# JGI-Bioinformatics/Kmernator

Hardware: AMD Instinct MI355X
Metric: total k-mers/sec at k=31, 150 bp reads (spectrum build, inputs resident in HBM) (higher is better)
Workload: dtype u64

## Files before the change

### kmernator_amd/csrc/kmr_api.hip

```cpp
#include <hip/hip_runtime.h>
#include <dlfcn.h>
#include <unistd.h>
#include <rccl/rccl.h>

#include <algorithm>
#include <atomic>
#include <cmath>
#include <cstdio>
#include <cstdlib>
#include <cstring>
#include <cctype>
#include <memory>
#include <mutex>
#include <string>
#include <type_traits>
#include <vector>

#include "kmr_host.hpp"
#include "kmr_kernels.hpp"
#include "kmr_partition.hpp"
#include "kmr_superkmer.hpp"
#include "kmr_buckets.hpp"
#include "kmr_synth.hpp"
#define KMR_INSTANCES_EXTERN
// ... 84 lines not shown
	HIPCHK(h, hipGetLastError());
	return 0;
}
int clear_table_any(kmr_handle *h, void *slots, ExtSlot *ext, uint32_t log2cap) { return with_w(h, [&](auto W) { return clear_table<W()>(h, slots, ext, log2cap); }); }

int alloc_table(kmr_handle *h, uint32_t log2cap, DevBuf &slots, DevBuf &ext) {
	DevBuf s, x;
	HIPCHK(h, s.alloc(slot_bytes(h) << log2cap));
	if (h->ext) HIPCHK(h, x.alloc(sizeof(ExtSlot) << log2cap));
	const int rc = clear_table_any(h, s.get(), x.get<ExtSlot>(), log2cap);
	if (rc) return rc;
	slots = std::move(s); ext = std::move(x);
	return 0;
}

int sync_state(kmr_handle *h) {
	HIPCHK(h, hipStreamSynchronize(h->stream));
	for (int which = 0; which < KMR_TIME_GROUPS; which++) {
		for (auto &pr : h->pending_events[which]) {
			float ms = 0; hipEventElapsedTime(&ms, pr.first, pr.second);
			h->ms[which] += ms; h->launches[which]++;
			hipEventDestroy(pr.first); hipEventDestroy(pr.second);
		}
		h->pending_events[which].clear();
	}
	uint32_t e = 0; DevStats s;
	HIPCHK(h, hipMemcpy(&e, h->derr.get<uint32_t>(), sizeof(e), hipMemcpyDeviceToHost));
	HIPCHK(h, hipMemcpy(&s, h->dstats.get<DevStats>(), sizeof(s), hipMemcpyDeviceToHost));
#ifdef KMR_DEBUG_HOOKS
	if (h->superkmer_mode) { if (dbg()) fprintf(stderr, "sk_extract windows: %llu general, %llu fast\n", s.claimed, s.inserted); s.claimed = 0; s.inserted = 0; }
#endif
	h->stats.raw_kmers = s.raw + s.inserted + s.sender_bad; h->stats.raw_good_kmers = s.good + s.inserted; h->stats.discarded = s.raw - s.good + s.sender_bad;
	h->occupied = s.claimed; h->pending_kmers = 0; h->subtracted = s.subtracted;
	if (e & ERR_READ_TOO_LONG) return fail(h, KMR_ERR_UNSUPPORTED, "a read is longer than the per-wavefront LDS tile (" + std::to_string(TILE_SPAN) + " bases)");
	if (e & ERR_TABLE_FULL) return fail(h, KMR_ERR_CAPACITY, "device k-mer table is full; raise kmr_config.max_table_entries / estimated_raw_kmers");
	if (e & ERR_SEGMENT_OVERFLOW) return fail(h, KMR_ERR_CAPACITY, "an owner segment overflowed seg_capacity");
	if (e & ERR_POOL_FULL) return fail(h, KMR_ERR_CAPACITY, "record pool overflow (internal sizing error)");
	if (e & ERR_ENTRIES_FULL) return fail(h, KMR_ERR_CAPACITY, "entry buffer overflow (internal sizing error)");
	return 0;
}

template <int W, bool EXT> int grow_table_t(kmr_handle *h, uint32_t newlog) {
	DevBuf ns, ne;
	int rc = alloc_table(h, newlog, ns, ne);
	if (rc) return rc;
	Table<W> src = table_of<W>(h), dst; dst.slots = ns.get<Slot<W>>(); dst.ext = ne.get<ExtSlot>(); dst.log2cap = newlog;
	hipLaunchKernelGGL((rehash_kernel<W, EXT>), dim3(grid_for(1ull << h->log2cap)), dim3(256), 0, h->stream, src, dst, h->hkb, h->derr.get<uint32_t>());
	HIPCHK(h, hipGetLastError());
	HIPCHK(h, hipStreamSynchronize(h->stream));
	h->slots = std::move(ns); h->extslots = std::move(ne); h->log2cap = newlog;
	return 0;
}
int grow_table(kmr_handle *h, uint32_t newlog) { return with_w_ext(h, [&](auto W, auto EXT) { return grow_table_t<W(), EXT()>(h, newlog); }); }

int ensure_capacity(kmr_handle *h, uint64_t incoming) {
	const uint64_t cap = 1ull << h->log2cap;
	if ((double)(h->occupied + h->pending_kmers + incoming) <= 0.85 * (double)cap) { h->pending_kmers += incoming; return 0; }
	int rc = sync_state(h);
	if (rc) return rc;
	if ((double)(h->occupied + incoming) > 0.85 * (double)cap) {
		uint32_t nl = h->log2cap;
		while ((double)(h->occupied + incoming) > 0.6 * (double)(1ull << nl)) nl++;
		rc = grow_table(h, nl);
		if (rc) return rc;
	}
	h->pending_kmers = incoming;
	return 0;
}

void time_begin(kmr_handle *h, int which, hipEvent_t *a, hipEvent_t *b) {
	hipEventCreate(a); hipEventCreate(b);
	hipEventRecord(*a, h->stream);
	(void)which;
}
void time_end(kmr_handle *h, int which, hipEvent_t a, hipEvent_t b) {
	hipEventRecord(b, h->stream);
	h->pending_events[which].push_back(std::make_pair(a, b));
}

const size_t EXTRACT_SMEM = (size_t)WAVES_PER_BLOCK * 2 * TILE_BUF;

int prepare_units(kmr_handle *h, ReadsView &rv, uint32_t span = (uint32_t)TILE_SPAN) {
	rv.u_start = rv.u_end = rv.u_read = nullptr; rv.n_units = 0;
	const uint64_t n = rv.n_reads;
	if (n == 0) return 0;
	int rc = h->umax.reserve(h, "umax", 4); if (rc) return rc;
	HIPCHK(h, hipMemsetAsync(h->umax.get<unsigned int>(), 0, 4, h->stream));
	rc = h->ucnt.reserve(h, "ucnt", 4 * (n + 1)); if (rc) return rc;
	hipLaunchKernelGGL(unit_count_kernel, dim3(grid_for(n)), dim3(256), 0, h->stream, rv.offsets, n, h->k, span, h->ucnt.get<uint32_t>(), h->umax.get<unsigned int>());
	HIPCHK(h, hipGetLastError());
	unsigned int mx = 0;
	HIPCHK(h, hipMemcpyAsync(&mx, h->umax.get<unsigned int>(), 4, hipMemcpyDeviceToHost, h->stream));
	HIPCHK(h, hipStreamSynchronize(h->stream));
	if (mx <= span) return 0;
	rc = h->ufirst.reserve(h, "ufirst", 8 * (n + 1)); if (rc) return rc;
	rc = exclusive_scan(h, h->ucnt.get<uint32_t>(), n, h->ufirst.get<uint64_t>()); if (rc) return rc;
	uint64_t U = 0;
	HIPCHK(h, hipMemcpy(&U, h->ufirst.get<uint64_t>() + n, 8, hipMemcpyDeviceToHost));
	if (h->u_read.cap() < 8 * U) {
		h->u_start.reset(); h->u_end.reset(); h->u_read.reset();
		HIPCHK(h, h->u_start.alloc(8 * U)); HIPCHK(h, h->u_end.alloc(8 * U)); HIPCHK(h, h->u_read.alloc(8 * U));
	}
	hipLaunchKernelGGL(unit_fill_kernel, dim3(grid_for(n)), dim3(256), 0, h->stream, rv.offsets, n, h->k, span, h->ufirst.get<uint64_t>(), h->u_start.get<uint64_t>(), h->u_end.get<uint64_t>(), h->u_read.get<uint64_t>());
	HIPCHK(h, hipGetLastError());
	rv.u_start = h->u_start.get<uint64_t>(); rv.u_end = h->u_end.get<uint64_t>(); rv.u_read = h->u_read.get<uint64_t>(); rv.n_units = U;
	return 0;
}

template <int W, bool EXT, class Op> int launch_extract(kmr_handle *h, const ReadsView &rv, const Op &op, uint64_t max_blocks = 0) {
	const DevParams dp = dev_params(h);
	const bool sub = Op::NEEDS_WEIGHT && (dp.sub_wnb | dp.sub_snb) != 0;
	auto kern = sub ? extract_kernel<W, EXT, Op, true> : extract_kernel<W, EXT, Op, false>;
	HIPCHK(h, hipFuncSetAttribute((const void *)kern, hipFuncAttributeMaxDynamicSharedMemorySize, (int)EXTRACT_SMEM));
	if (dbg()) { int nb = 0; hipOccupancyMaxActiveBlocksPerMultiprocessor(&nb, (const void *)kern, WAVES_PER_BLOCK * 64, EXTRACT_SMEM); fprintf(stderr, "extract: %d blocks of %d waves per CU (dynamic LDS %zu)\n", nb, WAVES_PER_BLOCK, EXTRACT_SMEM);
		for (size_t tr : {(size_t)79872, (size_t)65536, (size_t)52000, (size_t)38000}) { hipOccupancyMaxActiveBlocksPerMultiprocessor(&nb, (const void *)kern, WAVES_PER_BLOCK * 64, tr); fprintf(stderr, "   with %zu bytes: %d blocks\n", tr, nb); } }
	const uint64_t tiles = ((rv.u_start ? rv.n_units : rv.n_reads) + 63) / 64;
	uint64_t blocks = (tiles + WAVES_PER_BLOCK - 1) / WAVES_PER_BLOCK;
	if (blocks == 0) return 0;
	if (max_blocks && blocks > max_blocks) blocks = max_blocks;
	if (blocks > 0x7fffffffull) return fail(h, KMR_ERR_INVALID_ARG, "too many reads in one batch");
	hipLaunchKernelGGL(kern, dim3((unsigned)blocks), dim3(WAVES_PER_BLOCK * 64), EXTRACT_SMEM, h->stream, rv, dp, op);
	HIPCHK(h, hipGetLastError());
	return 0;
}

template <int W, bool EXT> int add_reads_dev_t(kmr_handle *h, const ReadsView &rvAll, uint64_t total_bases) {
	const uint64_t n = rvAll.n_reads;
	const uint64_t avg = n ? std::max<uint64_t>(1, total_bases / n) : 1;
	uint64_t chunk = std::max<uint64_t>(64, ((1ull << 27) / avg) & ~63ull);
	std::vector<uint64_t> off2(2);
	for (uint64_t r = 0; r < n; r += chunk) {
		const uint64_t m = std::min(chunk, n - r);
		HIPCHK(h, hipMemcpyAsync(&off2[0], rvAll.offsets + r, 8, hipMemcpyDeviceToHost, h->stream));
		HIPCHK(h, hipMemcpyAsync(&off2[1], rvAll.offsets + r + m, 8, hipMemcpyDeviceToHost, h->stream));
		HIPCHK(h, hipStreamSynchronize(h->stream));
		const uint64_t bases = off2[1] - off2[0];
		int rc = ensure_capacity(h, bases);
		if (rc) return rc;
		ReadsView rv = reads_slice(rvAll, r, m);
		rc = prepare_units(h, rv); if (rc) return rc;
		InsertOp<W, EXT> op; op.table = table_of<W>(h);
		hipEvent_t a, b; time_begin(h, 0, &a, &b);
		rc = launch_extract<W, EXT>(h, rv, op);
		time_end(h, 0, a, b);
		if (rc) return rc;
	}
	return 0;
}

int add_reads_dev_any(kmr_handle *h, const ReadsView &rv, uint64_t total_bases) { return with_w_ext(h, [&](auto W, auto EXT) { return add_reads_dev_t<W(), EXT()>(h, rv, total_bases); }); }

}
namespace kmr_host {
int exclusive_scan(kmr_handle *h, const uint32_t *in, uint64_t n, uint64_t *out ) {
	const uint64_t nblocks = (n + SCAN_ITEMS - 1) / SCAN_ITEMS;
	const size_t eb = sizeof(unsigned long long);
	int rc = h->scan_sums.reserve(h, "scan_sums", eb * (nblocks + 1), eb * std::max<uint64_t>(nblocks + 1, 4096)); if (rc) return rc;
	unsigned long long *sums = h->scan_sums.get<unsigned long long>(), *total = sums + nblocks;
	hipLaunchKernelGGL(scan_block_sums_kernel, dim3((unsigned)nblocks), dim3(256), 0, h->stream, in, n, sums);
	hipLaunchKernelGGL(scan_sums_kernel, dim3(1), dim3(256), 0, h->stream, sums, nblocks, total);
	hipLaunchKernelGGL(scan_apply_kernel, dim3((unsigned)nblocks), dim3(256), 0, h->stream, in, n, sums, out);
	HIPCHK(h, hipGetLastError());
	HIPCHK(h, hipStreamSynchronize(h->stream));
	return 0;
}
}
namespace {

int arena_alloc(kmr_handle *h, void **out, size_t bytes) {
	const size_t need = (bytes + 255) & ~(size_t)255;
	if (h->arena && h->arena_used + need <= h->arena.cap()) { *out = h->arena.get<uint8_t>() + h->arena_used; h->arena_used += need; h->arena_want += need; return 0; }
	h->arena_want += need;
	DevBuf b;
	HIPCHK(h, b.alloc(std::max<size_t>(need, 256)));
	*out = b.get();
	h->arena_overflow.push_back(std::move(b));
	return 0;
}
int arena_reset(kmr_handle *h) {
	HIPCHK(h, hipStreamSynchronize(h->stream));
	h->arena_overflow.clear();
	if (h->arena_want > h->arena.cap()) {
		if (h->arena.alloc(h->arena_want + h->arena_want / 8 + (1 << 20)) != hipSuccess) (void)hipGetLastError();
	}
	h->arena_used = 0; h->arena_want = 0;
	return 0;
}
template <class T> int arena_get(kmr_handle *h, T **out, size_t count) { return arena_alloc(h, (void **)out, count * sizeof(T)); }

void clear_map(DevMap &m) { m.image.reset(); m.n = 0; m.present = false; }


template <int W> MapView<W> view_of(const DevMap &m, uint32_t vw) {
	MapView<W> v; v.start = m.start.get<uint64_t>(); v.keys = m.keys.get<uint64_t>(); v.vals = m.vals.get<uint32_t>(); v.sweight = m.sweight.get<uint8_t>(); v.nb = m.present ? m.nb : 0; v.vw = vw;
	return v;
}

template <int W, bool EXT> int finalize_t(kmr_handle *h, uint32_t min_depth) {
	int rc = sync_state(h);
	if (rc) return rc;
	hipEvent_t ea, eb; time_begin(h, 1, &ea, &eb);
	const FinalizeParams f = finalize_params(h, min_depth);
	const bool keepSing = f.has_singletons && min_depth <= 1;
	DevBuf wcb, scb, fcb;
	HIPCHK(h, wcb.alloc(4 * h->nb_weak)); HIPCHK(h, scb.alloc(4 * h->nb_sing)); HIPCHK(h, fcb.alloc(sizeof(FinalizeCounters)));
	uint32_t *wc = wcb.get<uint32_t>(), *sc = scb.get<uint32_t>(); FinalizeCounters *fc = fcb.get<FinalizeCounters>();
	HIPCHK(h, hipMemsetAsync(wc, 0, 4 * h->nb_weak, h->stream)); HIPCHK(h, hipMemsetAsync(sc, 0, 4 * h->nb_sing, h->stream)); HIPCHK(h, hipMemsetAsync(fc, 0, sizeof(FinalizeCounters), h->stream));
	Table<W> t = table_of<W>(h);
	const int g = grid_for(1ull << h->log2cap);
	hipLaunchKernelGGL(classify_kernel<W>, dim3(g), dim3(256), 0, h->stream, t, f, wc, sc, fc);
	HIPCHK(h, hipGetLastError());
	FinalizeCounters c;
	HIPCHK(h, hipMemcpyAsync(&c, fc, sizeof(c), hipMemcpyDeviceToHost, h->stream));
	HIPCHK(h, hipStreamSynchronize(h->stream));
	h->stats.unique_kmers = c.unique;
	h->stats.singleton_kmers = f.has_singletons ? c.singletons : 0;
	DevMap &wm = h->weak, &sm = h->sing;
	wm = DevMap(); sm = DevMap();
	wm.nb = h->nb_weak; wm.n = c.weak_kept; wm.present = true;
	sm.nb = h->nb_sing; sm.n = c.sing_kept; sm.present = keepSing;
	const uint32_t vw = EXT ? 15 : 3;
	HIPCHK(h, wm.start.alloc(8 * (wm.nb + 1))); HIPCHK(h, sm.start.alloc(8 * (sm.nb + 1)));
	rc = exclusive_scan(h, wc, wm.nb, wm.start.get<uint64_t>()); if (rc) return rc;
	rc = exclusive_scan(h, sc, sm.nb, sm.start.get<uint64_t>()); if (rc) return rc;
	HIPCHK(h, wm.keys.alloc(std::max<uint64_t>(8, 8ull * W * wm.n))); HIPCHK(h, wm.vals.alloc(std::max<uint64_t>(8, 4ull * vw * wm.n)));
	HIPCHK(h, sm.keys.alloc(std::max<uint64_t>(8, 8ull * W * sm.n))); HIPCHK(h, sm.sweight.alloc(std::max<uint64_t>(8, sm.n)));
	if (EXT) HIPCHK(h, sm.spkt.alloc(std::max<uint64_t>(8, 4ull * sm.n)));
	HIPCHK(h, hipMemsetAsync(wc, 0, 4 * h->nb_weak, h->stream)); HIPCHK(h, hipMemsetAsync(sc, 0, 4 * h->nb_sing, h->stream));
	hipLaunchKernelGGL((scatter_kernel<W, EXT>), dim3(g), dim3(256), 0, h->stream, t, f, wm.start.get<uint64_t>(), wc, wm.keys.get<uint64_t>(), wm.vals.get<uint32_t>(), sm.start.get<uint64_t>(), sc, sm.keys.get<uint64_t>(), sm.sweight.get<uint8_t>(), sm.spkt.get<uint32_t>());
	HIPCHK(h, hipGetLastError());
	SortView<W> sv; sv.keys = wm.keys.get<uint64_t>(); sv.vals = wm.vals.get<uint32_t>(); sv.b8 = nullptr; sv.pkt = nullptr; sv.vw = vw;
	hipLaunchKernelGGL((sort_buckets_kernel<W, EXT ? 15 : 3>), dim3(grid_for(wm.nb, 4, 1 << 20)), dim3(256), 0, h->stream, sv, wm.start.get<uint64_t>(), wm.nb);
	if (sm.n) {
		SortView<W> ss; ss.keys = sm.keys.get<uint64_t>(); ss.vals = nullptr; ss.b8 = sm.sweight.get<uint8_t>(); ss.pkt = sm.spkt.get<uint32_t>(); ss.vw = 0;
		hipLaunchKernelGGL((sort_buckets_kernel<W, 0>), dim3(grid_for(sm.nb, 4, 1 << 20)), dim3(256), 0, h->stream, ss, sm.start.get<uint64_t>(), sm.nb);
	}
	HIPCHK(h, hipGetLastError());
	time_end(h, 1, ea, eb);
	HIPCHK(h, hipStreamSynchronize(h->stream));
	h->has_singletons = keepSing;
	if (!keepSing) { sm.n = 0; }
	h->stats.weak_entries = wm.n; h->stats.singleton_entries = keepSing ? sm.n : 0;
	h->finalized = true; h->map_gen++;
	return sync_state(h);
}

template <int W> int build_image_t(kmr_handle *h, DevMap &m, bool weakMap) {
	if (m.image) return 0;
	const uint32_t vw = h->ext ? 15 : 3;
	const uint32_t vbytes = weakMap ? (h->ext ? 60 : 12) : (h->ext ? 5 : 1);
	HIPCHK(h, m.image.alloc(8 * (2 + m.nb) + 4 * m.nb + m.n * (h->kb + vbytes)));
	hipLaunchKernelGGL(image_header_kernel, dim3(grid_for(m.nb)), dim3(256), 0, h->stream, m.image.get<uint8_t>(), m.start.get<uint64_t>(), m.nb, h->kb, vbytes);
	if (m.n) hipLaunchKernelGGL(image_entries_kernel<W>, dim3(grid_for(m.n)), dim3(256), 0, h->stream, m.image.get<uint8_t>(), m.start.get<uint64_t>(), m.nb, h->kb, vbytes,
	                           m.keys.get<uint64_t>(), weakMap ? m.vals.get<uint32_t>() : nullptr, vw, m.sweight.get<uint8_t>(), m.spkt.get<uint32_t>(), m.n);
	HIPCHK(h, hipGetLastError());
	HIPCHK(h, hipStreamSynchronize(h->stream));
	return 0;
}
int build_image(kmr_handle *h, DevMap &m, bool weakMap) { return with_w(h, [&](auto W) { return build_image_t<W()>(h, m, weakMap); }); }

template <int W> int load_image_t(kmr_handle *h, DevMap &m, bool weakMap, const uint8_t *src, uint64_t len) {
	if (len < 16) return fail(h, KMR_ERR_INVALID_ARG, "image too short");
	uint64_t nb, mask; memcpy(&nb, src, 8); memcpy(&mask, src + 8, 8);
	if (nb == 0 || (nb & (nb - 1)) || mask != nb - 1 || len < 8 * (2 + nb) + 4 * nb) return fail(h, KMR_ERR_INVALID_ARG, "bad image header");
	const uint32_t vw = h->ext ? 15 : 3;
	const uint32_t vbytes = weakMap ? (h->ext ? 60 : 12) : (h->ext ? 5 : 1);
	if ((len - 8 * (2 + nb) - 4 * nb) % (h->kb + vbytes) != 0) return fail(h, KMR_ERR_INVALID_ARG, "image size does not match k / value type");
	m = DevMap();
	m.nb = nb; m.n = (len - 8 * (2 + nb) - 4 * nb) / (h->kb + vbytes); m.present = true;
	const uint64_t *offs = (const uint64_t *)(src + 16);
	uint64_t expect = 8 * (2 + nb);
	for (uint64_t b = 0; b < nb; b++) {
		if (offs[b] != expect || expect + 4 > len) return fail(h, KMR_ERR_INVALID_ARG, "image offsets are not the packed store() layout");
		uint32_t cnt; memcpy(&cnt, src + expect, 4);
		expect += 4 + (uint64_t)cnt * (h->kb + vbytes);
		if (expect > len) return fail(h, KMR_ERR_INVALID_ARG, "image bucket runs past the end");
	}
	if (expect != len) return fail(h, KMR_ERR_INVALID_ARG, "image length mismatch");
	HIPCHK(h, m.image.alloc(len));
	HIPCHK(h, hipMemcpy(m.image.get<uint8_t>(), src, len, hipMemcpyHostToDevice));
	{
		DevBuf counts; HIPCHK(h, counts.alloc(4 * nb));
		hipLaunchKernelGGL(image_counts_kernel, dim3(grid_for(nb)), dim3(256), 0, h->stream, m.image.get<uint8_t>(), nb, counts.get<uint32_t>());
		HIPCHK(h, m.start.alloc(8 * (nb + 1)));
		int rc = exclusive_scan(h, counts.get<uint32_t>(), nb, m.start.get<uint64_t>()); if (rc) return rc;
	}
	HIPCHK(h, m.keys.alloc(std::max<uint64_t>(8, 8ull * W * m.n)));
	if (weakMap) HIPCHK(h, m.vals.alloc(std::max<uint64_t>(8, 4ull * vw * m.n)));
	else { HIPCHK(h, m.sweight.alloc(std::max<uint64_t>(8, m.n))); if (h->ext) HIPCHK(h, m.spkt.alloc(std::max<uint64_t>(8, 4 * m.n))); }
	if (m.n) hipLaunchKernelGGL(image_unpack_kernel<W>, dim3(grid_for(m.n)), dim3(256), 0, h->stream, m.image.get<uint8_t>(), m.start.get<uint64_t>(), nb, h->kb, vbytes, m.keys.get<uint64_t>(), m.vals.get<uint32_t>(), vw, m.sweight.get<uint8_t>(), m.spkt.get<uint32_t>(), m.n);
	SortView<W> sv; sv.keys = m.keys.get<uint64_t>(); sv.vals = m.vals.get<uint32_t>(); sv.b8 = m.sweight.get<uint8_t>(); sv.pkt = m.spkt.get<uint32_t>(); sv.vw = weakMap ? vw : 0;
	if (!weakMap) hipLaunchKernelGGL((sort_buckets_kernel<W, 0>), dim3(grid_for(nb, 4, 1 << 20)), dim3(256), 0, h->stream, sv, m.start.get<uint64_t>(), nb);
	else if (h->ext) hipLaunchKernelGGL((sort_buckets_kernel<W, 15>), dim3(grid_for(nb, 4, 1 << 20)), dim3(256), 0, h->stream, sv, m.start.get<uint64_t>(), nb);
	else hipLaunchKernelGGL((sort_buckets_kernel<W, 3>), dim3(grid_for(nb, 4, 1 << 20)), dim3(256), 0, h->stream, sv, m.start.get<uint64_t>(), nb);
	HIPCHK(h, hipGetLastError());
	HIPCHK(h, hipStreamSynchronize(h->stream));
	m.image.reset();

	return 0;
}

template <int W, int VW> void launch_sort(kmr_handle *h, DevMap &m, bool weakMap) {
	SortView<W> sv; sv.keys = m.keys.get<uint64_t>(); sv.vals = weakMap ? m.vals.get<uint32_t>() : nullptr; sv.b8 = m.sweight.get<uint8_t>(); sv.pkt = m.spkt.get<uint32_t>(); sv.vw = weakMap ? VW : 0;
	hipLaunchKernelGGL((sort_buckets_kernel<W, VW>), dim3(grid_for(m.nb, 4, 1 << 20)), dim3(256), 0, h->stream, sv, m.start.get<uint64_t>(), m.nb);
}
template <int W> int merge_image_t(kmr_handle *h, DevMap &m, bool weakMap, const uint8_t *src, uint64_t len) {
	DevMap t;
	int rc = load_image_t<W>(h, t, weakMap, src, len);
	if (rc) return rc;
	if (t.nb != m.nb) return fail(h, KMR_ERR_INVALID_ARG, "Can not merge two maps of differing sizes (src/Kmer.h:3210)");
	const uint32_t vw = h->ext ? 15 : 3;
	DevMap d; d.nb = m.nb; d.n = m.n + t.n; d.present = true;
	DevBuf countsb, dupb;
	HIPCHK(h, countsb.alloc(4 * m.nb)); HIPCHK(h, dupb.alloc(4));
	uint32_t *counts = countsb.get<uint32_t>(), *dup = dupb.get<uint32_t>();
// ... 198 lines not shown
				HIPCHK(h, hipStreamSynchronize(h->stream));
				h->uw_keys.reset(); h->uw_vals.reset(); h->us_keys.reset(); h->us_b8.reset(); h->us_pkt.reset(); h->ue.reset(); h->ue2.reset();
			}
		}
		uint64_t want = est / CH + launches * (uint64_t)grid * ((1ull << h->bits1) + 512) + 64 + l2_allowance;
		{
			size_t mfree = 0, mtotal = 0;
			const double twice = (double)(want + est / CH) * CH * rec_bytes(h) * 1.02;
			if (hipMemGetInfo(&mfree, &mtotal) == hipSuccess && twice + (double)(8ull << 30) < (double)mfree * 0.5) want += est / CH;
		}
		int rc0 = pool_reserve(h, h->l1, want, true);
		if (rc0) return rc0;
	}
	int rc = pool_reserve(h, h->l1, max_records / CH + (uint64_t)grid * ((1ull << h->bits1) + 512) + 64, true);
	if (rc) return rc;
	rc = zero_work_counter(h); if (rc) return rc;
	PartSource<W> S; memset(&S, 0, sizeof(S));
	S.linear = linear; S.ext_start = ext_start; S.ext_count = ext_count; S.n_ext = n_ext; S.ext_stride = ext_stride; S.ext_len = ext_len; S.total = total;
	S.valid_counter = valid_counter; S.kb = h->hkb; S.rot = part_rot(h); S.packed_words = packed_words; S.ordinal_base = ordinal_base;
	if (!h->tune.no_l1_state) {
		rc = ensure_l1_state<W, EXT>(h); if (rc) return rc;
		S.state = h->l1_state.get<uint8_t>(); S.state_final = 0; h->l1_state_dirty = true;
	}
	hipEvent_t ta, tb; time_begin(h, KMR_TIME_PARTITION1, &ta, &tb);
	rc = launch_partition<W, EXT, 1>(h, S, h->l1, grid, h->bits1, 0);
	time_end(h, KMR_TIME_PARTITION1, ta, tb);
	return rc;
}

void choose_bits1(kmr_handle *h, uint64_t records_hint) {
	uint64_t est = std::max<uint64_t>(records_hint, h->cfg.estimated_raw_kmers / std::max<uint32_t>(1, h->cfg.world_size));
	const int mb = max_part_bits(h);
	int T = 0; while (T < 2 * mb && (est >> T) > TARGET_LIST_RECORDS) T++;
	h->bits1 = std::max(0, std::min(mb, T + 2 - mb));
}

template <int W, bool EXT> int extract_by_owner_t(kmr_handle *h, const ReadsView &rvAll, uint64_t total_bases, void *dev_records, uint64_t seg_capacity, void *dev_seg_counts, uint32_t *dev_pos = nullptr) {
	const uint64_t n = rvAll.n_reads;
	const uint64_t avg = n ? std::max<uint64_t>(1, total_bases / n) : 1;
	const uint64_t chunk = std::max<uint64_t>(64, (SUB_BATCH_BASES / avg) & ~63ull);
	for (uint64_t r = 0; r < n; r += chunk) {
		const uint64_t m = std::min(chunk, n - r);
		ReadsView rv = reads_slice(rvAll, r, m);
		int rc = prepare_units(h, rv); if (rc) return rc;
		const uint64_t nu = rv.u_start ? rv.n_units : m;
		rc = h->kcap.reserve(h, "kcap", 4 * std::max<uint64_t>(nu + 1, 16)); if (rc) return rc;
		rc = h->koff.reserve(h, "koff", 8 * std::max<uint64_t>(nu + 1, 16)); if (rc) return rc;
		hipLaunchKernelGGL(kmer_capacity_kernel, dim3(grid_for(nu)), dim3(256), 0, h->stream, rv, h->k, h->kcap.get<uint32_t>());
		HIPCHK(h, hipGetLastError());
		rc = exclusive_scan(h, h->kcap.get<uint32_t>(), nu, h->koff.get<uint64_t>()); if (rc) return rc;
		uint64_t total_cap = 0;
		HIPCHK(h, hipMemcpy(&total_cap, h->koff.get<uint64_t>() + nu, 8, hipMemcpyDeviceToHost));
		const uint64_t tiles = (nu + 63) / 64;
		rc = h->linear.reserve(h, "linear", sizeof(typename PoolRec<W, EXT>::type) * std::max<uint64_t>(total_cap, 16)); if (rc) return rc;
		rc = h->tile_count.reserve(h, "tile_count", 4 * std::max<uint64_t>(tiles, 16)); if (rc) return rc;
		LinearOp<W, EXT, false> op; op.records = (typename PoolRec<W, EXT>::type *)h->linear.get(); op.koff = h->koff.get<uint64_t>(); op.tile_count = h->tile_count.get<uint32_t>(); op.first_read_idx = rv.first_read_idx;
		h->sender_launch = dev_pos == nullptr;
		rc = launch_extract<W, EXT>(h, rv, op);
		h->sender_launch = false;
		if (rc) return rc;
		rc = zero_work_counter(h); if (rc) return rc;
		const int grid = (int)std::min<uint64_t>((uint64_t)num_cus(h) * 8, tiles);
		OwnerFn of; of.m = 0; of.off = of.win = of.list_bits = 0;
		if (h->superkmer_mode && h->sk_exchange) { of.m = h->sk_m; of.off = h->sk_off; of.win = h->sk_win; of.list_bits = h->sk_bits; }
		if (dev_pos)
			hipLaunchKernelGGL((owner_scatter_kernel<W, EXT, true>), dim3(grid), dim3(OWNER_THREADS), 0, h->stream, (const typename PoolRec<W, EXT>::type *)h->linear.get(), h->koff.get<uint64_t>(), h->tile_count.get<uint32_t>(), tiles, h->hkb,
			                   h->cfg.world_size, (uint32_t *)dev_records, seg_capacity, (unsigned long long *)dev_seg_counts, h->work_counter.get<unsigned int>(), h->derr.get<uint32_t>(), dev_pos, of);
		else
			hipLaunchKernelGGL((owner_scatter_kernel<W, EXT>), dim3(grid), dim3(OWNER_THREADS), 0, h->stream, (const typename PoolRec<W, EXT>::type *)h->linear.get(), h->koff.get<uint64_t>(), h->tile_count.get<uint32_t>(), tiles, h->hkb,
			                   h->cfg.world_size, (uint32_t *)dev_records, seg_capacity, (unsigned long long *)dev_seg_counts, h->work_counter.get<unsigned int>(), h->derr.get<uint32_t>(), (uint32_t *)nullptr, of);
		HIPCHK(h, hipGetLastError());
	}
	return 0;
}

template <int W, bool EXT> int add_reads_partition_t(kmr_handle *h, const ReadsView &rvAll, uint64_t total_bases) {
	const uint64_t n = rvAll.n_reads;
	if (!h->l1.head) choose_bits1(h, total_bases);
	const uint64_t avg = n ? std::max<uint64_t>(1, total_bases / n) : 1;
	const uint64_t sub_bases = h->tune.sub_batch_bases ? h->tune.sub_batch_bases : SUB_BATCH_BASES;
	const uint64_t chunk = std::max<uint64_t>(64, (sub_bases / avg) & ~63ull);
	for (uint64_t r = 0; r < n; r += chunk) {
		const uint64_t m = std::min(chunk, n - r);
		ReadsView rv = reads_slice(rvAll, r, m);
		int rc = prepare_units(h, rv); if (rc) return rc;
		const uint64_t nu = rv.u_start ? rv.n_units : m;
		rc = h->kcap.reserve(h, "kcap", 4 * std::max<uint64_t>(nu + 1, 16)); if (rc) return rc;
		rc = h->koff.reserve(h, "koff", 8 * std::max<uint64_t>(nu + 1, 16)); if (rc) return rc;
		hipLaunchKernelGGL(kmer_capacity_kernel, dim3(grid_for(nu)), dim3(256), 0, h->stream, rv, h->k, h->kcap.get<uint32_t>());
		HIPCHK(h, hipGetLastError());
		rc = exclusive_scan(h, h->kcap.get<uint32_t>(), nu, h->koff.get<uint64_t>()); if (rc) return rc;
		uint64_t total_cap = 0;
		HIPCHK(h, hipMemcpy(&total_cap, h->koff.get<uint64_t>() + nu, 8, hipMemcpyDeviceToHost));
		const uint64_t tiles = (nu + 63) / 64;
		rc = h->linear.reserve(h, "linear", rec_bytes(h) * std::max<uint64_t>(total_cap, 16)); if (rc) return rc;
		rc = h->tile_count.reserve(h, "tile_count", 4 * std::max<uint64_t>(tiles, 16)); if (rc) return rc;
		LinearOp<W, EXT> op; op.records = (typename PoolRec<W, EXT>::type *)h->linear.get(); op.koff = h->koff.get<uint64_t>(); op.tile_count = h->tile_count.get<uint32_t>(); op.first_read_idx = rv.first_read_idx;
		hipEvent_t a, b, a2, b2; time_begin(h, KMR_TIME_BUILD, &a, &b);
		time_begin(h, KMR_TIME_EXTRACT, &a2, &b2);
		rc = launch_extract<W, EXT>(h, rv, op);
		time_end(h, KMR_TIME_EXTRACT, a2, b2);
#ifdef KMR_DEBUG_HOOKS
		if (!rc && getenv("KMR_DEBUG_SAME_TILE")) {
			const uint64_t distinct = std::max<uint64_t>(1, strtoull(getenv("KMR_DEBUG_SAME_TILE"), nullptr, 10));
			hipLaunchKernelGGL(same_tile_kernel, dim3(grid_for(tiles)), dim3(256), 0, h->stream, h->koff.get<uint64_t>(), tiles, distinct, total_cap / std::max<uint64_t>(tiles, 1));
		}
#endif
		if (!rc) rc = partition_level1<W, EXT>(h, h->linear.get(), h->koff.get<uint64_t>(), h->tile_count.get<uint32_t>(), tiles, 64, 0, 0, total_cap);
		time_end(h, KMR_TIME_BUILD, a, b);
		if (rc) return rc;
	}
	return 0;
}
int add_reads_partition(kmr_handle *h, const ReadsView &rv, uint64_t total_bases) { return with_w_ext(h, [&](auto W, auto EXT) { return add_reads_partition_t<W(), EXT()>(h, rv, total_bases); }); }

int build_csr(kmr_handle *h, HostPool &p, uint64_t nl, uint32_t first, uint64_t **list_start, uint64_t **list_chunks, uint32_t *n_chunks_out) {
	unsigned int used = 0;
	HIPCHK(h, hipStreamSynchronize(h->stream));
	HIPCHK(h, hipMemcpy(&used, p.head.get<unsigned int>(), 4, hipMemcpyDeviceToHost));
	if (used > p.cap) used = p.cap;
	used = used > first ? used - first : 0;
	uint32_t *cnt;
	{ int arc = arena_get(h, &cnt, nl); if (arc) return arc; arc = arena_get(h, list_start, nl + 1); if (arc) return arc;
	  arc = arena_get(h, list_chunks, std::max<unsigned>(used, 1)); if (arc) return arc; }
	HIPCHK(h, hipMemsetAsync(cnt, 0, 4 * nl, h->stream));
	const unsigned csr_grid = (unsigned)(((uint64_t)used + CSR_THREADS * CSR_ITEMS - 1) / (CSR_THREADS * CSR_ITEMS));
	if (used) hipLaunchKernelGGL(chunk_hist_kernel, dim3(csr_grid), dim3(CSR_THREADS), 0, h->stream, p.chunk_list.get<uint32_t>() + first, used, cnt, (uint32_t)nl);
	int rc = exclusive_scan(h, cnt, nl, *list_start); if (rc) return rc;
	HIPCHK(h, hipMemsetAsync(cnt, 0, 4 * nl, h->stream));
	if (used) hipLaunchKernelGGL(chunk_scatter_kernel, dim3(csr_grid), dim3(CSR_THREADS), 0, h->stream, p.chunk_list.get<uint32_t>() + first, p.chunk_count.get<uint32_t>() + first, used, first, *list_start, cnt, *list_chunks, (uint32_t)nl);
	HIPCHK(h, hipGetLastError());
	*n_chunks_out = used;
	if (dbg()) {
		unsigned long long hv[2] = {0, 0};
		DevBuf db; HIPCHK(h, db.alloc(16)); HIPCHK(h, hipMemset(db.get(), 0, 16));
		unsigned long long *d = db.get<unsigned long long>();
		if (used) hipLaunchKernelGGL(pool_records_kernel, dim3(grid_for(used)), dim3(256), 0, h->stream, p.chunk_list.get<uint32_t>(), p.chunk_count.get<uint32_t>(), used, d, d + 1);
		HIPCHK(h, hipStreamSynchronize(h->stream));
		HIPCHK(h, hipMemcpy(hv, d, 16, hipMemcpyDeviceToHost));
		fprintf(stderr, "build_csr: lists %llu chunks %u valid %llu records %llu (expected %llu)\n", (unsigned long long)nl, used, hv[1], hv[0], (unsigned long long)h->stats.raw_good_kmers);
		unsigned long long vv[3] = {0, 0, 0};
		int bits = 0; while ((1ull << bits) < nl) bits++;
		DevBuf vb; HIPCHK(h, vb.alloc(24)); HIPCHK(h, hipMemset(vb.get(), 0, 24));
		unsigned long long *v = vb.get<unsigned long long>();
		PoolView pvw = pool_view(h, p);
		with_w_ext(h, [&](auto W, auto EXT) { hipLaunchKernelGGL((verify_lists_kernel<W(), EXT()>), dim3(4096), dim3(256), 0, h->stream, pvw, *list_start, *list_chunks, nl, bits, h->hkb, part_rot(h), v, v + 1, v + 2); });
		HIPCHK(h, hipStreamSynchronize(h->stream));
		HIPCHK(h, hipMemcpy(vv, v, 24, hipMemcpyDeviceToHost));
		fprintf(stderr, "verify_lists: records via CSR %llu misfiled %llu zero-weight %llu\n", vv[0], vv[1], vv[2]);
	}
	return 0;
}

int finish_maps_from_entries(kmr_handle *h, uint32_t *wc, uint32_t *sc, uint64_t wslots, uint64_t sslots, uint64_t wn, uint64_t sn, bool keepSing, bool weak_uncounted = false);
CountOut count_out(kmr_handle *h, bool packed, unsigned long long *cursors, uint32_t *wc, uint32_t *sc, FinalizeCounters *fc);

template <int W, bool EXT, int LOG2S, bool NARROW = false> int launch_count(kmr_handle *h, int grid, const uint64_t *ls, const uint64_t *lc, uint64_t nl, const CountOut &out, const FinalizeParams &f, int list_filter) {
	auto kern = count_kernel<W, EXT, LOG2S, NARROW>;
	const size_t smem = count_smem_bytes<W, EXT, LOG2S, NARROW>();
	HIPCHK(h, hipFuncSetAttribute((const void *)kern, hipFuncAttributeMaxDynamicSharedMemorySize, (int)smem));
	hipLaunchKernelGGL(kern, dim3(grid), dim3(COUNT_THREADS), smem, h->stream, pool_view(h, h->l1), ls, lc, nl, out, f, h->work_counter.get<unsigned int>(), list_filter);
	return 0;
}

template <int W, bool EXT> int finalize_partition_t(kmr_handle *h, uint32_t min_depth) {
	int rc = sync_state(h);
	if (rc) return rc;
	hipEvent_t ea, eb; time_begin(h, 1, &ea, &eb);
	const uint64_t G = h->stats.raw_good_kmers;
	const FinalizeParams f = finalize_params(h, min_depth);
	const bool keepSing = f.has_singletons && min_depth <= 1;
	if (!h->l1.head) { rc = pool_reserve(h, h->l1, 0, false); if (rc) return rc; }
	rc = arena_reset(h); if (rc) return rc;
	rc = flush_l1_state<W, EXT>(h); if (rc) return rc;
	const uint64_t nl1 = 1ull << h->bits1;
	uint64_t *ls1 = nullptr; uint64_t *lc1 = nullptr; uint32_t nch1 = 0;
	rc = build_csr(h, h->l1, nl1, 0, &ls1, &lc1, &nch1); if (rc) return rc;
	double distinct_share = 1.0, repeated_share = 0.5;
	if (G) {
		unsigned long long *dpr, hpr[4] = {0, 0, 0, 0};
		const uint32_t n_probes = (uint32_t)std::min<uint64_t>(PROBE_LISTS, nl1);
		const size_t tbytes = 8 * ((size_t)n_probes * PROBE_SLOTS + 4);
		rc = arena_alloc(h, (void **)&dpr, tbytes); if (rc) return rc;
		HIPCHK(h, hipMemsetAsync(dpr, 0, tbytes, h->stream));
		hipLaunchKernelGGL((distinct_probe_kernel<W, EXT>), dim3(n_probes * PROBE_SPLIT), dim3(256), 0, h->stream, pool_view(h, h->l1), ls1, lc1, nl1, h->hkb, part_rot(h),
		                   (int)h->bits1, n_probes, dpr + 4, dpr);
		HIPCHK(h, hipGetLastError());
		HIPCHK(h, hipMemcpyAsync(hpr, dpr, 32, hipMemcpyDeviceToHost, h->stream)); HIPCHK(h, hipStreamSynchronize(h->stream));
		if (hpr[0] >= 256) { distinct_share = std::min(1.0, std::max(0.01, (double)hpr[1] / (double)hpr[0])); repeated_share = std::min(0.5, (double)hpr[2] / (double)hpr[0]); }
		if (dbg()) fprintf(stderr, "distinct probe: %llu records, %llu distinct (%llu repeated) -> shares %.3f %.3f\n", hpr[0], hpr[1], hpr[2], distinct_share, repeated_share);
	}
	const int mb = max_part_bits(h);
	int T = 0; while (T < 40 && ((G >> T) > TARGET_LIST_RECORDS || (double)(G >> T) * distinct_share > MAX_LIST_DISTINCT)) T++;
	T = std::min(T, 28);
	int cur_bits = h->bits1;
	uint64_t *ls2 = ls1, *lc2 = lc1;
	uint32_t valid_from = 0;
	for (int level = 2; cur_bits < T; level++) {
		const int nbits = std::min(mb, T - cur_bits);
		const uint64_t nl_prev = 1ull << cur_bits;
		std::vector<uint64_t> hs(nl_prev + 1);
		HIPCHK(h, hipMemcpy(hs.data(), ls2, 8 * (nl_prev + 1), hipMemcpyDeviceToHost));
		std::vector<uint64_t> ib, ie; std::vector<uint32_t> il;
		for (uint64_t l = 0; l < nl_prev; l++) {
			const uint64_t nch = hs[l + 1] - hs[l];
			if (!nch) continue;
			const uint64_t nit = (nch + L2_ITEM_CHUNKS - 1) / L2_ITEM_CHUNKS, per = (nch + nit - 1) / nit;
			for (uint64_t c = hs[l]; c < hs[l + 1]; c += per) { ib.push_back(c); ie.push_back(std::min(hs[l + 1], c + per)); il.push_back((uint32_t)l); }
		}
		if (ib.empty()) { cur_bits += nbits; rc = build_csr(h, h->l1, 1ull << cur_bits, valid_from, &ls2, &lc2, &nch1); if (rc) return rc; continue; }
		const uint64_t partials = ib.size() * (1ull << nbits) + (uint64_t)part_grid(h) * 512 + 64;
		unsigned int head_before = 0;
		HIPCHK(h, hipMemcpy(&head_before, h->l1.head.get<unsigned int>(), 4, hipMemcpyDeviceToHost));
		const bool recycle = h->tune.recycle >= 0 ? h->tune.recycle != 0 : (uint64_t)head_before + G / CH + partials + 64 > h->l1.cap;
		h->l1.used_ub = head_before;
		rc = pool_reserve(h, h->l1, (recycle ? 0 : G / CH) + partials, true); if (rc) return rc;
		uint64_t *dib, *die; uint32_t *dil;
		rc = arena_get(h, &dib, ib.size()); if (rc) return rc; rc = arena_get(h, &die, ie.size()); if (rc) return rc; rc = arena_get(h, &dil, il.size()); if (rc) return rc;
		HIPCHK(h, hipMemcpyAsync(dib, ib.data(), 8 * ib.size(), hipMemcpyHostToDevice, h->stream)); HIPCHK(h, hipMemcpyAsync(die, ie.data(), 8 * ie.size(), hipMemcpyHostToDevice, h->stream));
		HIPCHK(h, hipMemcpyAsync(dil, il.data(), 4 * il.size(), hipMemcpyHostToDevice, h->stream));
		rc = zero_work_counter(h); if (rc) return rc;
		PartSource<W> S; memset(&S, 0, sizeof(S));
		S.src = pool_view(h, h->l1); S.list_chunks = lc2; S.item_begin = dib; S.item_end = die; S.item_list = dil; S.n_items = ib.size(); S.kb = h->hkb; S.rot = part_rot(h);
		S.recycle = recycle ? 1 : 0;
		const int grid = (int)std::min<uint64_t>(partition_blocks(h), ib.size());
		if (dbg()) fprintf(stderr, "level %d: %d bits after %d, %zu items, %s\n", level, nbits, cur_bits, ib.size(), recycle ? "recycling chunks" : "fresh chunks");
		hipEvent_t ta, tb; time_begin(h, KMR_TIME_PARTITION2, &ta, &tb);
		rc = launch_partition<W, EXT, 2>(h, S, h->l1, grid, nbits, cur_bits);
		time_end(h, KMR_TIME_PARTITION2, ta, tb);
		if (rc) return rc;
		HIPCHK(h, hipStreamSynchronize(h->stream));
		cur_bits += nbits;
		if (!recycle) valid_from = head_before;
		rc = build_csr(h, h->l1, 1ull << cur_bits, valid_from, &ls2, &lc2, &nch1); if (rc) return rc;
	}
	const uint64_t nl2 = 1ull << cur_bits;
	const int count_log2s = (!EXT && (double)(G >> cur_bits) * distinct_share > MAX_LIST_DISTINCT) ? 11 : COUNT_LOG2S;
	if (dbg()) fprintf(stderr, "count pass: %llu lists of ~%llu records, table 2^%d\n", (unsigned long long)nl2, (unsigned long long)(G >> cur_bits), count_log2s);
	const uint32_t vw = EXT ? 15 : 3;
	const uint64_t slack = (uint64_t)part_grid(h) * 8 * 8192 + 16;
	const uint64_t wbound = f.has_singletons ? G / 2 : G, sbound = keepSing ? G : 0;
	const uint64_t wmax = wbound + wbound / 8 + slack, smax = keepSing ? sbound + sbound / 8 + slack : 16;
	uint64_t wcap = std::min<uint64_t>(wmax, (uint64_t)((double)G * (f.has_singletons ? repeated_share : distinct_share) * 1.5) + G / 64 + slack);
	uint64_t scap = keepSing ? std::min<uint64_t>(smax, (uint64_t)((double)G * std::max(0.0, distinct_share - repeated_share) * 1.5) + G / 64 + slack) : 16;
	if (h->tune.entry_share >= 0) {
		const double sh = h->tune.entry_share;
		wcap = std::min<uint64_t>(wmax, (uint64_t)((double)G * sh) + 16384); if (keepSing) scap = std::min<uint64_t>(smax, (uint64_t)((double)G * sh) + 16384);
		h->uw_keys.reset(); h->uw_vals.reset(); h->us_keys.reset(); h->us_b8.reset(); h->us_pkt.reset();
	}
	wcap = std::max(wcap, key_entries(h, h->uw_keys)); scap = std::max(scap, key_entries(h, h->us_keys));
	uint32_t *wc = nullptr, *sc = nullptr; FinalizeCounters *fc = nullptr; unsigned long long *cursors = nullptr;
	rc = arena_get(h, &wc, h->nb_weak); if (rc) return rc; rc = arena_get(h, &sc, h->nb_sing); if (rc) return rc;
	rc = arena_get(h, &fc, 1); if (rc) return rc; rc = arena_get(h, &cursors, 2); if (rc) return rc;
	FinalizeCounters c; unsigned long long cur[2];
	hipEvent_t tca, tcb; time_begin(h, KMR_TIME_COUNT, &tca, &tcb);
	for (int attempt = 0; ; attempt++) {
	{
		const double need = (key_entries(h, h->uw_keys) < wcap ? (8.0 * W + 4.0 * vw) * (double)wcap : 0.0) + (key_entries(h, h->us_keys) < scap ? (8.0 * W + 1.0) * (double)scap : 0.0);
		size_t mfree = 0, mtotal = 0;
		if (need > 0 && h->linear && hipMemGetInfo(&mfree, &mtotal) == hipSuccess && (double)mfree < need + (double)G * 0.3 * (8.0 * W + 12.0) + (double)(2ull << 30)) {
			HIPCHK(h, hipStreamSynchronize(h->stream));
			h->linear.reset();
		}
	}
	if (key_entries(h, h->uw_keys) < wcap || !h->uw_vals) {
		h->uw_keys.reset(); h->uw_vals.reset();
		HIPCHK(h, h->uw_keys.alloc(8ull * W * wcap)); HIPCHK(h, h->uw_vals.alloc(4ull * vw * wcap));
	}
	if (key_entries(h, h->us_keys) < scap || !h->us_b8 || (EXT && !h->us_pkt)) {
		h->us_keys.reset(); h->us_b8.reset(); h->us_pkt.reset();
		HIPCHK(h, h->us_keys.alloc(8ull * W * scap)); HIPCHK(h, h->us_b8.alloc(scap)); if (EXT) HIPCHK(h, h->us_pkt.alloc(4 * scap));
	}
	HIPCHK(h, hipMemsetAsync(wc, 0, 4 * h->nb_weak, h->stream)); HIPCHK(h, hipMemsetAsync(sc, 0, 4 * h->nb_sing, h->stream));
	HIPCHK(h, hipMemsetAsync(fc, 0, sizeof(FinalizeCounters), h->stream)); HIPCHK(h, hipMemsetAsync(cursors, 0, 16, h->stream));
	const CountOut out = count_out(h, false, cursors, wc, sc, fc);
	rc = zero_work_counter(h); if (rc) return rc;
	#ifdef KMR_DEBUG_HOOKS
	const int count_reps = getenv("KMR_COUNT_CHECK") ? atoi(getenv("KMR_COUNT_CHECK")) : 0;
#else
	const int count_reps = 0;
#endif
	for (int cr = 0; cr <= count_reps; cr++) {
		if (cr) {
			FinalizeCounters c0; unsigned long long cur0[2];
			HIPCHK(h, hipStreamSynchronize(h->stream));
			HIPCHK(h, hipMemcpy(&c0, fc, sizeof(c0), hipMemcpyDeviceToHost)); HIPCHK(h, hipMemcpy(cur0, cursors, 16, hipMemcpyDeviceToHost));
			fprintf(stderr, "count pass %d: unique %llu singletons %llu weak_kept %llu sing_kept %llu slots %llu/%llu\n", cr - 1, (unsigned long long)c0.unique,
			        (unsigned long long)c0.singletons, (unsigned long long)c0.weak_kept, (unsigned long long)c0.sing_kept, cur0[0], cur0[1]);
			HIPCHK(h, hipMemsetAsync(wc, 0, 4 * h->nb_weak, h->stream)); HIPCHK(h, hipMemsetAsync(sc, 0, 4 * h->nb_sing, h->stream));
			HIPCHK(h, hipMemsetAsync(fc, 0, sizeof(FinalizeCounters), h->stream)); HIPCHK(h, hipMemsetAsync(cursors, 0, 16, h->stream));
			rc = zero_work_counter(h); if (rc) return rc;
		}
		const int grid = (int)std::min<uint64_t>((uint64_t)part_grid(h) * 2, nl2);
		if (count_log2s == 11) {
			rc = launch_count<W, EXT, 11>(h, grid, ls2, lc2, nl2, out, f, 0); if (rc) return rc;
		} else if (EXT && W == 1 && !h->tune.no_narrow) {
			rc = launch_count<W, EXT, COUNT_LOG2S, true>(h, grid, ls2, lc2, nl2, out, f, 1); if (rc) return rc;
			HIPCHK(h, hipGetLastError());
			rc = zero_work_counter(h); if (rc) return rc;
			hipLaunchKernelGGL(max_list_chunks_kernel, dim3(grid_for(nl2)), dim3(256), 0, h->stream, ls2, nl2, h->work_counter.get<unsigned int>());
			unsigned int longest = 0;
			HIPCHK(h, hipMemcpyAsync(&longest, h->work_counter.get<unsigned int>(), 4, hipMemcpyDeviceToHost, h->stream));
			HIPCHK(h, hipStreamSynchronize(h->stream));
			rc = zero_work_counter(h); if (rc) return rc;
			if (longest > COUNT_NARROW_CHUNKS) { rc = launch_count<W, EXT, COUNT_LOG2S>(h, std::min(grid, part_grid(h)), ls2, lc2, nl2, out, f, 2); if (rc) return rc; }
		} else {
			rc = launch_count<W, EXT, COUNT_LOG2S>(h, grid, ls2, lc2, nl2, out, f, 0); if (rc) return rc;
		}
		HIPCHK(h, hipGetLastError());
	}
	uint32_t cerr = 0;
	HIPCHK(h, hipMemcpyAsync(&c, fc, sizeof(c), hipMemcpyDeviceToHost, h->stream)); HIPCHK(h, hipMemcpyAsync(cur, cursors, 16, hipMemcpyDeviceToHost, h->stream));
	HIPCHK(h, hipMemcpyAsync(&cerr, h->derr.get<uint32_t>(), 4, hipMemcpyDeviceToHost, h->stream));
	HIPCHK(h, hipStreamSynchronize(h->stream));
	if (!(cerr & ERR_ENTRIES_FULL) || (wcap >= wmax && scap >= smax) || attempt >= 8) break;
	cerr &= ~(uint32_t)ERR_ENTRIES_FULL;
	HIPCHK(h, hipMemcpy(h->derr.get<uint32_t>(), &cerr, 4, hipMemcpyHostToDevice));
	wcap = std::min<uint64_t>(wmax, wcap * 2); if (keepSing) scap = std::min<uint64_t>(smax, scap * 2);
	if (dbg()) fprintf(stderr, "count pass: entry buffers too small, retrying with %llu / %llu\n", (unsigned long long)wcap, (unsigned long long)scap);
	}
	time_end(h, KMR_TIME_COUNT, tca, tcb);
	{
		uint32_t cerr2 = 0;
		HIPCHK(h, hipMemcpy(&cerr2, h->derr.get<uint32_t>(), 4, hipMemcpyDeviceToHost));
		if (cerr2 & ERR_ENTRIES_FULL) { time_end(h, 1, ea, eb); return fail(h, KMR_ERR_CAPACITY, "entry buffers of the count pass overflowed at their upper bound (internal sizing error)"); }
	}

	h->stats.unique_kmers = c.unique;
	h->stats.singleton_kmers = f.has_singletons ? c.singletons : 0;
	hipEvent_t tma, tmb; time_begin(h, KMR_TIME_BUCKETS, &tma, &tmb);
	rc = finish_maps_from_entries(h, wc, sc, cur[0], cur[1], c.weak_kept, c.sing_kept, keepSing);
	time_end(h, KMR_TIME_BUCKETS, tma, tmb);
	if (rc) return rc;
	time_end(h, 1, ea, eb);
	h->has_singletons = keepSing;
	h->stats.weak_entries = h->weak.n; h->stats.singleton_entries = keepSing ? h->sing.n : 0;
	h->finalized = true; h->map_gen++;
	rc = sync_state(h);
	if (!rc && !h->arena_overflow.empty()) rc = arena_reset(h);
	return rc;
}

template <int W> int binned_buckets_t(kmr_handle *h, uint64_t wslots, uint64_t wn, bool &done) {
	done = false;
	DevMap &wm = h->weak;
	const uint64_t nb = wm.nb;
	uint32_t B = 0; while ((1ull << (B + 1)) <= nb) B++;
	if (h->ext || wn < h->tune.binned_min || wn == 0 || (1ull << B) != nb || wslots >= (1ull << 40)) return 0;
	uint32_t g = 0; while (g < std::min<uint32_t>(B, BB_MAX_GROUP_BITS) && (wn >> (B - g)) < 512) g++;
	const uint32_t R = B - g;
	if (R < 1 || R > 2 * BB_MAX_BITS || (wn >> R) > 1024) return 0;
	const uint32_t bits1 = R <= (uint32_t)BB_MAX_BITS ? R : (R + 1) / 2, bits2 = R - bits1;
	const uint64_t bins1 = 1ull << bits1, groups = 1ull << R;
	uint32_t *hist1 = nullptr, *hist2 = nullptr, *pad1 = nullptr; uint64_t *start1 = nullptr, *gstart = nullptr; unsigned long long *cursor = nullptr; unsigned int *dmax = nullptr;
	int rc = arena_get(h, &hist1, bins1); if (rc) return rc;
	rc = arena_get(h, &start1, bins1 + 1); if (rc) return rc;
	rc = arena_get(h, &cursor, groups); if (rc) return rc;
	rc = arena_get(h, &dmax, 1); if (rc) return rc;
	if (bits2) { rc = arena_get(h, &hist2, groups); if (rc) return rc; rc = arena_get(h, &pad1, bins1); if (rc) return rc; rc = arena_get(h, &gstart, groups + 1); if (rc) return rc; }
	HIPCHK(h, hipMemsetAsync(hist1, 0, 4 * bins1, h->stream)); HIPCHK(h, hipMemsetAsync(dmax, 0, 4, h->stream));
	BbInput in1; in1.entries = h->ue.get<uint64_t>(); in1.seg_start = nullptr; in1.seg_count = nullptr; in1.n_seg = 1; in1.n_slots = wslots; in1.holes = 1;
	auto hist_grid = [&](uint64_t n_slots, uint32_t &tpb) { const uint64_t tiles = (n_slots + BB_TILE - 1) / BB_TILE; tpb = (uint32_t)std::max<uint64_t>(1, (tiles + 2047) / 2048); return (unsigned)((tiles + tpb - 1) / tpb); };
	auto scatter_grid = [&](uint64_t n_slots) { const uint64_t tiles = (n_slots + BB_TILE - 1) / BB_TILE; return (unsigned)std::min<uint64_t>(tiles, (uint64_t)num_cus(h) * 8); };
	auto scratch = [&](uint64_t entries) { return h->ue2.reserve(h, "ue2", 8ull * (W + 1) * entries); };
	auto group_launch = [&](const uint64_t *entries, const uint64_t *gs, const uint32_t *gc) -> int {
		int rc2 = wm.keys.reserve(h, "weak map keys", std::max<uint64_t>(8ull * W * wn, 8)); if (rc2) return rc2;
		rc2 = wm.vals.reserve(h, "weak map vals", std::max<uint64_t>(12ull * wn, 8)); if (rc2) return rc2;
		auto gk = bb_group_kernel<W>;
		HIPCHK(h, hipFuncSetAttribute((const void *)gk, hipFuncAttributeMaxDynamicSharedMemorySize, (int)bb_group_smem_bytes<W>()));
		int per_cu = 0;
		if (hipOccupancyMaxActiveBlocksPerMultiprocessor(&per_cu, (const void *)gk, BB_GROUP_THREADS, bb_group_smem_bytes<W>()) != hipSuccess || per_cu < 1) per_cu = 4;
		if (dbg()) fprintf(stderr, "bb_group<W=%d>: %d blocks per CU, %llu groups\n", W, per_cu, (unsigned long long)groups);
		hipLaunchKernelGGL(gk, dim3((unsigned)std::min<uint64_t>(groups, (uint64_t)num_cus(h) * per_cu)), dim3(BB_GROUP_THREADS), bb_group_smem_bytes<W>(), h->stream, entries, wm.keys.get<uint64_t>(), wm.vals.get<uint32_t>(), gs, gc, groups, g, h->hkb, nb, wm.start.get<uint64_t>(), wn, h->derr.get<uint32_t>());
		HIPCHK(h, hipGetLastError());
		return 0;
	};
	const uint32_t shift1 = B - bits1;
	uint32_t tpb = 1; unsigned grid = hist_grid(wslots, tpb);
	hipLaunchKernelGGL(bb_hist_kernel<W>, dim3(grid), dim3(BB_THREADS), 0, h->stream, in1, shift1, bits1, h->hkb, nb, tpb, hist1);
	unsigned int mx = 0;
	if (!bits2) {
		hipLaunchKernelGGL(bb_pad_kernel, dim3(grid_for(bins1)), dim3(256), 0, h->stream, (const uint32_t *)hist1, bins1, (uint32_t *)nullptr, dmax);
		HIPCHK(h, hipMemcpyAsync(&mx, dmax, 4, hipMemcpyDeviceToHost, h->stream));
		rc = exclusive_scan(h, hist1, bins1, start1); if (rc) return rc;
		if (mx > bb_group_cap<W>()) return 0;
		rc = scratch(wn); if (rc) return rc;
		hipLaunchKernelGGL(bb_cursor_init_kernel, dim3(grid_for(bins1)), dim3(256), 0, h->stream, (const uint64_t *)start1, bins1, cursor);
		hipLaunchKernelGGL(bb_scatter_kernel<W>, dim3(scatter_grid(wslots)), dim3(BB_THREADS), 0, h->stream, in1, shift1, bits1, h->hkb, nb, cursor, h->ue2.get<uint64_t>());
		rc = group_launch(h->ue2.get<uint64_t>(), start1, hist1); if (rc) return rc;
		done = true;
		return 0;
	}
	hipLaunchKernelGGL(bb_pad_kernel, dim3(grid_for(bins1)), dim3(256), 0, h->stream, (const uint32_t *)hist1, bins1, pad1, dmax);
	rc = exclusive_scan(h, pad1, bins1, start1); if (rc) return rc;
	uint64_t padded_total = 0;
	HIPCHK(h, hipMemcpy(&padded_total, start1 + bins1, 8, hipMemcpyDeviceToHost));
	rc = scratch(std::max(padded_total, wn)); if (rc) return rc;
	hipLaunchKernelGGL(bb_cursor_init_kernel, dim3(grid_for(bins1)), dim3(256), 0, h->stream, (const uint64_t *)start1, bins1, cursor);
	hipLaunchKernelGGL(bb_scatter_kernel<W>, dim3(scatter_grid(wslots)), dim3(BB_THREADS), 0, h->stream, in1, shift1, bits1, h->hkb, nb, cursor, h->ue2.get<uint64_t>());
	BbInput in2; in2.entries = h->ue2.get<uint64_t>(); in2.seg_start = start1; in2.seg_count = hist1; in2.n_seg = (uint32_t)bins1; in2.n_slots = padded_total; in2.holes = 0;
	const uint32_t shift2 = g;
	HIPCHK(h, hipMemsetAsync(hist2, 0, 4 * groups, h->stream)); HIPCHK(h, hipMemsetAsync(dmax, 0, 4, h->stream));
	grid = hist_grid(padded_total, tpb);
	hipLaunchKernelGGL(bb_hist_kernel<W>, dim3(grid), dim3(BB_THREADS), 0, h->stream, in2, shift2, bits2, h->hkb, nb, tpb, hist2);
	hipLaunchKernelGGL(bb_pad_kernel, dim3(grid_for(groups)), dim3(256), 0, h->stream, (const uint32_t *)hist2, groups, (uint32_t *)nullptr, dmax);
	HIPCHK(h, hipMemcpyAsync(&mx, dmax, 4, hipMemcpyDeviceToHost, h->stream));
	rc = exclusive_scan(h, hist2, groups, gstart); if (rc) return rc;
	if (mx > bb_group_cap<W>() || packed_entries(h, h->ue) < wn) return 0;
	hipLaunchKernelGGL(bb_cursor_init_kernel, dim3(grid_for(groups)), dim3(256), 0, h->stream, (const uint64_t *)gstart, groups, cursor);
	hipLaunchKernelGGL(bb_scatter_kernel<W>, dim3(scatter_grid(padded_total)), dim3(BB_THREADS), 0, h->stream, in2, shift2, bits2, h->hkb, nb, cursor, h->ue.get<uint64_t>());
	rc = group_launch(h->ue.get<uint64_t>(), gstart, hist2); if (rc) return rc;
	done = true;
	return 0;
}

template <int W> int finish_maps_t(kmr_handle *h, uint32_t *wc, uint32_t *sc, uint64_t wslots, uint64_t sslots, uint64_t wn, uint64_t sn, bool keepSing, bool weak_uncounted) {
	const uint32_t vw = h->ext ? 15 : 3;
	DevMap &wm = h->weak, &sm = h->sing;
	clear_map(wm); clear_map(sm);
	wm.nb = h->nb_weak; wm.n = wn; wm.present = true;
	sm.nb = h->nb_sing; sm.n = keepSing ? sn : 0; sm.present = keepSing;
	int rc = wm.start.reserve(h, "weak map start", 8 * (wm.nb + 1)); if (rc) return rc;
	rc = sm.start.reserve(h, "singleton map start", 8 * (sm.nb + 1)); if (rc) return rc;
	bool weakDone = false;
	if (weak_uncounted) {
		rc = binned_buckets_t<W>(h, wslots, wn, weakDone); if (rc) return rc;
		if (!weakDone) {
			if (key_entries(h, h->uw_keys) < wslots || !h->uw_vals) {
				h->uw_keys.reset(); h->uw_vals.reset();
				const uint64_t cap = std::max<uint64_t>(wslots, 16);
				HIPCHK(h, h->uw_keys.alloc(8ull * W * cap)); HIPCHK(h, h->uw_vals.alloc(12ull * cap));
			}
			HIPCHK(h, hipMemsetAsync(wc, 0, 4 * wm.nb, h->stream));
			if (wslots) hipLaunchKernelGGL(bb_unpack_kernel<W>, dim3(grid_for(wslots)), dim3(256), 0, h->stream, (const uint64_t *)h->ue.get<uint64_t>(), wslots, h->hkb, wm.nb, (uint64_t *)h->uw_keys.get(), (uint32_t *)h->uw_vals.get(), wc);
			HIPCHK(h, hipGetLastError());
		}
	}
	if (!weakDone) { rc = exclusive_scan(h, wc, wm.nb, wm.start.get<uint64_t>()); if (rc) return rc; }
	if (keepSing) { rc = exclusive_scan(h, sc, sm.nb, sm.start.get<uint64_t>()); if (rc) return rc; }
	else HIPCHK(h, hipMemsetAsync(sm.start.get<uint64_t>(), 0, 8 * (sm.nb + 1), h->stream));
	if (!weakDone) {
		rc = wm.keys.reserve(h, "weak map keys", std::max<uint64_t>(8ull * W * wm.n, 8)); if (rc) return rc;
		rc = wm.vals.reserve(h, "weak map vals", std::max<uint64_t>(4ull * vw * wm.n, 8)); if (rc) return rc;
	}
	rc = sm.keys.reserve(h, "singleton map keys", std::max<uint64_t>(8ull * W * sm.n, 8)); if (rc) return rc;
	rc = sm.sweight.reserve(h, "singleton map sweight", std::max<uint64_t>(sm.n, 8)); if (rc) return rc;
	if (h->ext) { rc = sm.spkt.reserve(h, "singleton map spkt", std::max<uint64_t>(4 * sm.n, 8)); if (rc) return rc; }
	HIPCHK(h, hipMemsetAsync(wc, 0, 4 * wm.nb, h->stream)); HIPCHK(h, hipMemsetAsync(sc, 0, 4 * sm.nb, h->stream));
	if (weakDone) {  }
	else if (wm.n && vw > 4) hipLaunchKernelGGL((entry_scatter_kernel<W, true>), dim3(grid_for(wslots)), dim3(256), 0, h->stream, (const uint64_t *)h->uw_keys.get(), (const uint32_t *)h->uw_vals.get(),
	                            (const uint8_t *)nullptr, (const uint32_t *)nullptr, wslots, vw, h->hkb, wm.nb, wm.start.get<uint64_t>(), wc, wm.keys.get<uint64_t>(), wm.vals.get<uint32_t>(), (uint8_t *)nullptr, (uint32_t *)nullptr);
	else if (wm.n) {
		unsigned long long *cur64 = nullptr;
		if (h->superkmer_mode && arena_get(h, &cur64, wm.nb) == 0) HIPCHK(h, hipMemcpyAsync(cur64, wm.start.get<uint64_t>(), 8 * wm.nb, hipMemcpyDeviceToDevice, h->stream));
		else cur64 = nullptr;
		hipLaunchKernelGGL(entry_scatter_kernel<W>, dim3(grid_for(wslots)), dim3(256), 0, h->stream, (const uint64_t *)h->uw_keys.get(), (const uint32_t *)h->uw_vals.get(),
		                            (const uint8_t *)nullptr, (const uint32_t *)nullptr, wslots, vw, h->hkb, wm.nb, wm.start.get<uint64_t>(), wc, wm.keys.get<uint64_t>(), wm.vals.get<uint32_t>(), (uint8_t *)nullptr, (uint32_t *)nullptr, cur64, 6);
	}
	if (sm.n) hipLaunchKernelGGL(entry_scatter_kernel<W>, dim3(grid_for(sslots)), dim3(256), 0, h->stream, (const uint64_t *)h->us_keys.get(), (const uint32_t *)nullptr,
	                            (const uint8_t *)h->us_b8.get(), (const uint32_t *)h->us_pkt.get(), sslots, 0u, h->hkb, sm.nb, sm.start.get<uint64_t>(), sc, sm.keys.get<uint64_t>(), (uint32_t *)nullptr, sm.sweight.get<uint8_t>(), h->ext ? sm.spkt.get<uint32_t>() : (uint32_t *)nullptr);
	HIPCHK(h, hipGetLastError());
	SortView<W> sv; sv.keys = wm.keys.get<uint64_t>(); sv.vals = wm.vals.get<uint32_t>(); sv.b8 = nullptr; sv.pkt = nullptr; sv.vw = vw;
	if (weakDone) {  }
	else if (h->ext) hipLaunchKernelGGL((sort_buckets_kernel<W, 15>), dim3(grid_for(wm.nb, 4, 1 << 20)), dim3(256), 0, h->stream, sv, wm.start.get<uint64_t>(), wm.nb);
	else hipLaunchKernelGGL((sort_buckets_kernel<W, 3>), dim3(grid_for(wm.nb, 4, 1 << 20)), dim3(256), 0, h->stream, sv, wm.start.get<uint64_t>(), wm.nb);
	if (sm.n) {
		SortView<W> ss; ss.keys = sm.keys.get<uint64_t>(); ss.vals = nullptr; ss.b8 = sm.sweight.get<uint8_t>(); ss.pkt = h->ext ? sm.spkt.get<uint32_t>() : nullptr; ss.vw = 0;
		hipLaunchKernelGGL((sort_buckets_kernel<W, 0>), dim3(grid_for(sm.nb, 4, 1 << 20)), dim3(256), 0, h->stream, ss, sm.start.get<uint64_t>(), sm.nb);
	}
	HIPCHK(h, hipGetLastError());
	HIPCHK(h, hipStreamSynchronize(h->stream));
	return 0;
}
int finish_maps_from_entries(kmr_handle *h, uint32_t *wc, uint32_t *sc, uint64_t wslots, uint64_t sslots, uint64_t wn, uint64_t sn, bool keepSing, bool weak_uncounted) {
	return with_w(h, [&](auto W) { return finish_maps_t<W()>(h, wc, sc, wslots, sslots, wn, sn, keepSing, weak_uncounted); });
}
int finalize_partition(kmr_handle *h, uint32_t min_depth) { return with_w_ext(h, [&](auto W, auto EXT) { return finalize_partition_t<W(), EXT()>(h, min_depth); }); }
template <int W, bool EXT> int insert_records_partition_t(kmr_handle *h, const void *recs, uint64_t n) {
	if (!h->l1.head) choose_bits1(h, n);
	hipEvent_t a, b; time_begin(h, 0, &a, &b);
	int rc = partition_level1<W, EXT>(h, recs, nullptr, nullptr, (n + 8191) / 8192, 0, 8192, n, n, &h->dstats.get<DevStats>()->inserted,
	                             2 * W + (h->ext ? 2 : 1), h->stream_base);
	time_end(h, 0, a, b);
	return rc;
}
int insert_records_partition(kmr_handle *h, const void *recs, uint64_t n) { return with_w_ext(h, [&](auto W, auto EXT) { return insert_records_partition_t<W(), EXT()>(h, recs, n); }); }
bool sk_geometry(uint32_t k, uint32_t m_wish, uint32_t &win, uint32_t &m, uint32_t &off, uint32_t win_max = 16) {
	for (uint32_t w : {32u, 16u, 8u, 4u}) {
		if (w > win_max) continue;
		if (w == 32u && (k < 45u || (m_wish && m_wish < 14u))) continue;
		if (k < w + 9) continue;
		uint32_t mm = std::min<uint32_t>(m_wish ? m_wish : 16u, k - w + 1);
		if (mm > 16) mm = 16;
		if (((k - mm + 1 - w) & 1u) != 0) mm--;
		if (mm < 10 && !m_wish) continue;
		if (mm < 4) continue;
		win = w; m = mm; off = (k - mm + 1 - w) / 2;
		return true;
	}
	return false;
}
const uint64_t SK_EXTRACT_WAVES_PER_CU = std::max(2 * SK_WAVES, SKL_MIN_BLOCKS * SKL_WAVES);
template <int W, int WIN, bool FILT, bool EXT = false> int launch_sk_extract(kmr_handle *h, const ReadsView &rv, const SkParams &sp, const DevParams *override_params = nullptr) {
	auto kern = sk_extract_kernel<W, WIN, FILT, EXT>;
	HIPCHK(h, hipFuncSetAttribute((const void *)kern, hipFuncAttributeMaxDynamicSharedMemorySize, (int)SK_EXTRACT_SMEM));
	const uint64_t tiles = ((rv.u_start ? rv.n_units : rv.n_reads) + 63) / 64;
	uint64_t blocks = (tiles + SK_WAVES - 1) / SK_WAVES;
	if (blocks == 0) return 0;
	blocks = std::min<uint64_t>(blocks, (uint64_t)num_cus(h) * 2);
	if (dbg()) { int nb = 0; hipOccupancyMaxActiveBlocksPerMultiprocessor(&nb, (const void *)kern, SK_WAVES * 64, SK_EXTRACT_SMEM); fprintf(stderr, "sk_extract<W=%d,WIN=%d>: %d blocks of %d waves per CU (LDS %zu), grid %llu, m=%u off=%u bits=%u\n", W, WIN, nb, SK_WAVES, SK_EXTRACT_SMEM, (unsigned long long)blocks, sp.m, sp.off, sp.list_bits); }
	hipLaunchKernelGGL(kern, dim3((unsigned)blocks), dim3(SK_WAVES * 64), SK_EXTRACT_SMEM, h->stream, rv, override_params ? *override_params : dev_params(h), sp, pool_view(h, h->l1));
	HIPCHK(h, hipGetLastError());
	return 0;
}
uint32_t sk_dbg_flags(const char *name);
bool sp_debug_extract(kmr_handle *h) { (void)h; return sk_dbg_flags("KMR_SK_EXTRACT_DBG") != 0; }
template <int W, int WIN, bool PACKED = false> int launch_sk_extract_lean(kmr_handle *h, const ReadsView &rv, const SkParams &sp, float wK, const DevParams *override_params = nullptr, const SkPacked *packed = nullptr) {
	auto kern = sk_extract_lean_kernel<W, WIN, PACKED>;
	SkPacked pkd{};
	if (PACKED) pkd = *packed;
	HIPCHK(h, hipFuncSetAttribute((const void *)kern, hipFuncAttributeMaxDynamicSharedMemorySize, (int)SKL_EXTRACT_SMEM));
	const uint64_t tiles = ((rv.u_start ? rv.n_units : rv.n_reads) + 63) / 64;
	uint64_t blocks = (tiles + SKL_WAVES - 1) / SKL_WAVES;
	if (blocks == 0) return 0;
	blocks = std::min<uint64_t>(blocks, (uint64_t)num_cus(h) * SKL_MIN_BLOCKS);
	hipLaunchKernelGGL(kern, dim3((unsigned)blocks), dim3(SKL_WAVES * 64), SKL_EXTRACT_SMEM, h->stream, rv, override_params ? *override_params : dev_params(h), sp, pool_view(h, h->l1), wK, pkd);
	HIPCHK(h, hipGetLastError());
	return 0;
}
int sk_uniform_weight(kmr_handle *h, const ReadsView &rv, bool &lean, float &wK) {
	lean = false; wK = 1.0f;
	if (h->tune.no_lean_extract) return 0;
	if (!rv.quals && h->uniform_q_hint < 0) { lean = true; return 0; }
	if (h->qual_mixed || rv.n_reads == 0) return 0;
	if (h->uniform_q_hint >= 0) {
		const unsigned int q0 = (unsigned int)h->uniform_q_hint;
		if (q0 == 127) { lean = true; wK = 1.0f; return 0; }
		if (!(h->hP[q0] > 0.0)) return 0;
		lean = true; wK = (float)h->hPk[q0];
		return 0;
	}
	{ int rc = h->qrange.reserve(h, "qrange", 8); if (rc) return rc; }
	const unsigned int init[2] = {255u, 0u};
	HIPCHK(h, hipMemcpyAsync(h->qrange.get<unsigned int>(), init, 8, hipMemcpyHostToDevice, h->stream));
	hipLaunchKernelGGL(sk_qual_range_kernel, dim3(num_cus(h) * 8), dim3(256), 0, h->stream, rv.quals, rv.offsets, rv.n_reads, h->qrange.get<unsigned int>());
	HIPCHK(h, hipGetLastError());
	unsigned int got[2] = {0, 0};
	HIPCHK(h, hipMemcpyAsync(got, h->qrange.get<unsigned int>(), 8, hipMemcpyDeviceToHost, h->stream));
	HIPCHK(h, hipStreamSynchronize(h->stream));
	if (got[0] != got[1]) { h->qual_mixed = got[0] < got[1]; return 0; }
	const unsigned int q0 = got[0];
	if (q0 == 127) { lean = true; wK = 1.0f; return 0; }
	if (!(h->hP[q0] > 0.0)) return 0;
	lean = true; wK = (float)h->hPk[q0];
	return 0;
}
uint32_t sk_dbg_flags(const char *name) {
#ifdef KMR_DEBUG_HOOKS
	const char *e = getenv(name); return e ? (uint32_t)atoi(e) : 0u;
#else
	(void)name; return 0u;
#endif
}
SkParams sk_params(kmr_handle *h) { SkParams sp; sp.dbg = sk_dbg_flags("KMR_SK_EXTRACT_DBG"); sp.keep_all_owners = h->sk_exchange ? 1u : 0u; sp.track = nullptr; sp.m = h->sk_m; sp.off = h->sk_off; sp.list_bits = h->sk_bits; sp.state = h->sk_state.get<unsigned long long>(); sp.Pk = h->dPk.get<double>(); sp.Rp = h->dPk.get<double>() + 256; sp.fast_div = h->sk_fast_div ? 1u : 0u; return sp; }
template <int W> int add_reads_superkmer_t(kmr_handle *h, const ReadsView &rvAll, uint64_t total_bases) {
	const uint64_t n = rvAll.n_reads;
	const DevParams dp = dev_params(h);
	const bool filt = dp.subsample > 1 || dp.num_parts > 1 || (dp.sub_wnb | dp.sub_snb) != 0 || (dp.world > 1 && !h->sk_exchange);
	bool lean = false; float wK = 1.0f;
	if (!filt && !h->ext && !sp_debug_extract(h)) { int rcq = sk_uniform_weight(h, rvAll, lean, wK); if (rcq) return rcq; }
	if (h->packed_direct && (!lean || h->cfg.size_tracker)) return fail(h, KMR_ERR_STATE, "internal: a packed batch handed to an extraction that wants text");
	if (rvAll.n_reads) {
		uint32_t wb; memcpy(&wb, &wK, 4);
		if (!lean) h->sk_uni_mixed = true;
		else if (h->sk_uni_w == SK_UNI_NONE) h->sk_uni_w = wb;
		else if (h->sk_uni_w != wb) h->sk_uni_mixed = true;
	}
	if (!h->sk_state) {
		const uint64_t est = h->cfg.estimated_raw_kmers ? h->cfg.estimated_raw_kmers : std::max<uint64_t>(total_bases, h->call_bases_hint) * std::max<uint32_t>(1, h->cfg.world_size);
		const uint64_t per_list = h->ext ? (W > 1 ? 400 : 600) : ((h->tune.target_list == 2048 && W > 1) ? 700 : h->tune.target_list * 3 / 4);
		uint32_t bits = 6; while (bits < 24 && (est >> bits) > per_list) bits++;
		h->sk_fine_shift = 0;
		if (h->sk_exchange && h->cfg.world_size > 1 && !h->tune.no_coarse_lists) {
			uint32_t sh = 0; while ((1u << sh) < h->cfg.world_size) sh++;
			if (bits >= 6 + sh) { h->sk_fine_shift = sh; bits -= sh; }
		}
		h->sk_bits = bits;
		if (h->cfg.world_size <= 1 && !h->sk_exchange && h->tune.target_list == 2048 && !h->tune.pow2_lists) {
			const uint64_t aim = h->tune.list_aim ? h->tune.list_aim : (W == 1 ? (h->ext ? 800 : (lean ? 1450 : 1700)) : per_list * 19 / 20);
			const uint64_t nlists = (est / aim + 63) & ~63ull;
			if (nlists > 64 && (nlists < (1ull << bits) || h->tune.list_aim) && nlists < (1ull << 31)) h->sk_bits = (uint32_t)nlists;
		}
		const uint64_t nl0 = sk_list_count(h->sk_bits);
		HIPCHK(h, h->sk_state.alloc(8 * nl0));
		hipLaunchKernelGGL(sk_state_init_kernel, dim3(grid_for(nl0)), dim3(256), 0, h->stream, h->sk_state.get<unsigned long long>(), nl0);
		HIPCHK(h, hipGetLastError());
	}
	const uint64_t avg = n ? std::max<uint64_t>(1, total_bases / n) : 1;
	const uint64_t sub_bases = h->tune.sub_batch_bases ? h->tune.sub_batch_bases : (1ull << 31);
	const uint64_t chunk = std::max<uint64_t>(64, (sub_bases / avg) & ~63ull);
	if (h->cfg.size_tracker && n) {
		h->trk_n = 0;
		{ int rc = h->trk.reserve(h, "trk", n * sizeof(SkTrackRec)); if (rc) return rc; }
		HIPCHK(h, hipMemsetAsync(h->trk.get<SkTrackRec>(), 0, n * sizeof(SkTrackRec), h->stream));
	}
	for (uint64_t r = 0; r < n; r += chunk) {
		const uint64_t m = std::min(chunk, n - r);
		ReadsView rv = reads_slice(rvAll, r, m);
		int rc = prepare_units(h, rv, h->packed_direct ? SK_PACKED_SPAN : (uint32_t)TILE_SPAN); if (rc) return rc;
		const uint64_t bases = m * avg + avg;
		if (!h->l1.base && r == 0 && h->cfg.world_size <= 1 && !h->sk_exchange && (h->cfg.estimated_raw_kmers || h->call_bases_hint > total_bases)) {
			const double job_bases = h->cfg.estimated_raw_kmers ? (double)h->cfg.estimated_raw_kmers * (double)avg / (double)(avg > h->k ? avg - h->k + 1 : 1) : (double)h->call_bases_hint;
			const double rest = job_bases - (double)total_bases;
			size_t fr = 0, tot = 0;
			if (rest > 0 && hipMemGetInfo(&fr, &tot) == hipSuccess) {
				const uint64_t want = (uint64_t)(rest * (h->ext ? 2.0 : 1.0) * (lean ? 0.3 : 0.65) / SK_CHUNK_G);
				h->l1.presize = std::min<uint64_t>(want, (uint64_t)(fr / 4) / ((size_t)CH * rec_bytes(h)));
			}
		}
		rc = pool_reserve(h, h->l1, (h->ext ? 2 : 1) * bases / SK_CHUNK_G + ((h->l1.base && !h->sk_exchange) ? 0 : sk_list_count(h->sk_bits)) + (uint64_t)num_cus(h) * SK_EXTRACT_WAVES_PER_CU * 130 + 64, true); if (rc) return rc;
		hipEvent_t a, b, a2, b2; time_begin(h, KMR_TIME_BUILD, &a, &b); time_begin(h, KMR_TIME_EXTRACT, &a2, &b2);
		SkParams sp = sk_params(h);
		if (h->cfg.size_tracker) sp.track = h->trk.get<SkTrackRec>() + r;
		if (h->packed_direct) {
			SkPacked pkd = *h->packed_direct; pkd.off += r; if (pkd.mk_off) pkd.mk_off += r;
			rc = with_win<W>(h->sk_win, [&](auto WIN) { return launch_sk_extract_lean<W, WIN(), true>(h, rv, sp, wK, nullptr, &pkd); });
		} else rc = with_win<W>(h->sk_win, [&](auto WIN) {
			if (h->ext) return filt ? launch_sk_extract<W, WIN(), true, true>(h, rv, sp) : launch_sk_extract<W, WIN(), false, true>(h, rv, sp);
// ... 276 lines not shown
		uint64_t first = h->early.hi;
		if (stride0 > 1) first += (first0 + stride0 - first % stride0) % stride0;
		p.lgMain.list_first = first;
	} else { h->early.active = false; memset(&early_c, 0, sizeof(early_c)); }
	return 0;
}
template <int W> int sk_long_items(kmr_handle *h, SkFinalize<W> &p) {
	p.lgItems = p.lgMain; p.n_items = 0;
	const uint64_t LONG_CHUNKS = p.ext ? std::min<uint64_t>(h->tune.long_list_chunks ? h->tune.long_list_chunks : SK_EXT_LONG_CHUNKS, SK_EXT_LONG_CHUNKS) : (h->tune.long_list_chunks ? h->tune.long_list_chunks : 1024), PIECE = std::max<uint64_t>(1, LONG_CHUNKS / 2);
	if (p.tracking || p.nch <= LONG_CHUNKS) return 0;
	const uint64_t cap = (uint64_t)p.nch / PIECE + 2 * 1024 + 16;
	uint64_t *ic0 = nullptr, *ic1 = nullptr; unsigned long long *dn = nullptr;
	int rc = arena_get(h, &ic0, cap); if (rc) return rc; rc = arena_get(h, &ic1, cap); if (rc) return rc; rc = arena_get(h, &dn, 1); if (rc) return rc;
	HIPCHK(h, hipMemsetAsync(dn, 0, 8, h->stream));
	hipLaunchKernelGGL(sk_long_items_kernel, dim3(grid_for(p.nl)), dim3(256), 0, h->stream, p.ls, p.nl, LONG_CHUNKS, PIECE, ic0, ic1, cap, dn);
	HIPCHK(h, hipGetLastError());
	unsigned long long hn = 0;
	HIPCHK(h, hipMemcpyAsync(&hn, dn, 8, hipMemcpyDeviceToHost, h->stream)); HIPCHK(h, hipStreamSynchronize(h->stream));
	if (hn > cap) return fail(h, KMR_ERR_CAPACITY, "long-list work items (internal sizing error)");
	p.n_items = hn;
	if (p.n_items) {
		p.lgMain.long_threshold = LONG_CHUNKS;
		p.lgItems.item_c0 = ic0; p.lgItems.item_c1 = ic1; p.lgItems.n_items = p.n_items; p.lgItems.merge_used = dn;
	}
	return 0;
}
CountOut count_out(kmr_handle *h, bool packed, unsigned long long *cursors, uint32_t *wc, uint32_t *sc, FinalizeCounters *fc) {
	CountOut out{};
	if (packed) { out.wentries = h->ue.get<uint64_t>(); out.wcap = packed_entries(h, h->ue); }
	else { out.wkeys = h->uw_keys.get<uint64_t>(); out.wvals = h->uw_vals.get<uint32_t>(); out.wcap = key_entries(h, h->uw_keys); out.spkt = h->us_pkt.get<uint32_t>(); out.weakCount = wc; }
	out.wcursor = cursors; out.scursor = cursors + 1;
	out.skeys = h->us_keys.get<uint64_t>(); out.sweight = h->us_b8.get<uint8_t>(); out.scap = key_entries(h, h->us_keys);
	out.singCount = sc; out.fc = fc; out.err = h->derr.get<uint32_t>();
	return out;
}
template <int W> int sk_count_pass(kmr_handle *h, SkFinalize<W> &p, bool &overflowed) {
	overflowed = false;
	const bool ext = p.ext, keepSing = p.keepSing, tracking = p.tracking; const uint32_t vw = ext ? 15 : 3;
	uint64_t &wcap = p.wcap, &scap = p.scap; const uint64_t wmax = p.wmax, smax = p.smax, nl = p.nl, n_items = p.n_items;
	uint32_t *wc = p.wc, *sc = p.sc; FinalizeCounters *fc = p.fc; unsigned long long *cursors = p.cursors;
	FinalizeCounters &c = p.c; unsigned long long *cur = p.cur; const SkTrackView &tv = p.tv; const FinalizeParams &f = p.f;
	int rc = 0;
	uint32_t merge_log2 = 16;
	hipEvent_t tca, tcb; time_begin(h, KMR_TIME_COUNT, &tca, &tcb);
	for (int attempt = 0; ; attempt++) {
		if (!ext && packed_entries(h, h->ue) < wcap) { h->ue.reset(); HIPCHK(h, h->ue.alloc(8ull * (W + 1) * wcap)); }
		if (ext && (key_entries(h, h->uw_keys) < wcap || !h->uw_vals)) {
			h->uw_keys.reset(); h->uw_vals.reset();
			HIPCHK(h, h->uw_keys.alloc(8ull * W * wcap)); HIPCHK(h, h->uw_vals.alloc(4ull * vw * wcap));
		}
		if (key_entries(h, h->us_keys) < scap || !h->us_b8 || (ext && !h->us_pkt)) {
			h->us_keys.reset(); h->us_b8.reset(); h->us_pkt.reset();
			HIPCHK(h, h->us_keys.alloc(8ull * W * scap)); HIPCHK(h, h->us_b8.alloc(scap)); if (ext) HIPCHK(h, h->us_pkt.alloc(4 * scap));
		}
		HIPCHK(h, hipMemsetAsync(wc, 0, 4 * h->nb_weak, h->stream)); HIPCHK(h, hipMemsetAsync(sc, 0, 4 * h->nb_sing, h->stream));
		HIPCHK(h, hipMemsetAsync(fc, 0, sizeof(FinalizeCounters), h->stream)); HIPCHK(h, hipMemsetAsync(cursors, 0, 16, h->stream));
		const CountOut out = count_out(h, !ext, cursors, wc, sc, fc);
		rc = zero_work_counter(h); if (rc) return rc;
		const int grid = (int)std::min<uint64_t>((uint64_t)num_cus(h) * 4, (nl / p.lgMain.list_stride + SK_LBATCH) / SK_LBATCH);
		SkCountLaunch<W> k;
		rc = sk_count_select<W>(h, ext, tracking, p.uni, k); if (rc) return rc;
		if (tracking) HIPCHK(h, hipMemsetAsync(tv.d_unique, 0, 8 * (tv.n + 1), h->stream));
		if (dbg()) { int nb = 0; hipOccupancyMaxActiveBlocksPerMultiprocessor(&nb, (const void *)k.kern, SKC_THREADS, k.smem); fprintf(stderr, "sk_count<W=%d>: %d blocks per CU (LDS %zu), %llu lists, %u chunks\n", W, nb, k.smem, (unsigned long long)nl, p.nch); }
		hipLaunchKernelGGL(k.kern, dim3(grid), dim3(SKC_THREADS), k.smem, h->stream, pool_view(h, h->l1), p.ls, p.lc, nl, h->k, out, f, h->work_counter.get<unsigned int>(), sk_dbg_flags("KMR_SK_COUNT_DBG"), tv, p.lgMain);
		HIPCHK(h, hipGetLastError());
		DevBuf mslots, mext;
		if (n_items) {
			SkLong<W> &lgItems = p.lgItems;
			if (mslots.alloc(sizeof(Slot<W>) << merge_log2) != hipSuccess) return fail(h, KMR_ERR_OOM, "merge table of the long lists");
			if (ext && mext.alloc(sizeof(ExtSlot) << merge_log2) != hipSuccess) return fail(h, KMR_ERR_OOM, "merge table of the long lists");
			hipLaunchKernelGGL(table_clear_kernel<W>, dim3(grid_for(1ull << merge_log2)), dim3(256), 0, h->stream, mslots.get<Slot<W>>(), mext.get<ExtSlot>(), 1ull << merge_log2);
			lgItems.merge.slots = mslots.get<Slot<W>>(); lgItems.merge.ext = mext.get<ExtSlot>(); lgItems.merge.log2cap = merge_log2;
			HIPCHK(h, hipMemsetAsync(lgItems.merge_used, 0, 8, h->stream));
			rc = zero_work_counter(h); if (rc) return rc;
			const int grid2 = (int)std::min<uint64_t>((uint64_t)num_cus(h) * 4, n_items);
			hipLaunchKernelGGL(k.kern, dim3(grid2), dim3(SKC_THREADS), k.smem, h->stream, pool_view(h, h->l1), p.ls, p.lc, nl, h->k, out, f, h->work_counter.get<unsigned int>(), sk_dbg_flags("KMR_SK_COUNT_DBG"), tv, lgItems);
			hipLaunchKernelGGL(sk_merge_emit_kernel<W>, dim3(grid_for(1ull << merge_log2)), dim3(256), 0, h->stream, lgItems.merge, out, f);
			if (hipGetLastError() != hipSuccess) return fail(h, KMR_ERR_HIP, "long-list launches");
		}
		uint32_t cerr = 0;
		HIPCHK(h, hipMemcpyAsync(&c, fc, sizeof(c), hipMemcpyDeviceToHost, h->stream)); HIPCHK(h, hipMemcpyAsync(cur, cursors, 16, hipMemcpyDeviceToHost, h->stream));
		HIPCHK(h, hipMemcpyAsync(&cerr, h->derr.get<uint32_t>(), 4, hipMemcpyDeviceToHost, h->stream));
		HIPCHK(h, hipStreamSynchronize(h->stream));
		if (n_items && (cerr & ERR_TABLE_FULL) && merge_log2 < 30) {
			cerr &= ~(uint32_t)(ERR_TABLE_FULL | ERR_ENTRIES_FULL);
			HIPCHK(h, hipMemcpy(h->derr.get<uint32_t>(), &cerr, 4, hipMemcpyHostToDevice));
			merge_log2 += 3;
			continue;
		}
		if (!(cerr & ERR_ENTRIES_FULL)) break;
		if ((wcap >= wmax && scap >= smax) || attempt >= 8) { overflowed = true; break; }
		cerr &= ~(uint32_t)ERR_ENTRIES_FULL;
		HIPCHK(h, hipMemcpy(h->derr.get<uint32_t>(), &cerr, 4, hipMemcpyHostToDevice));
		wcap = std::min<uint64_t>(wmax, wcap * 2); if (keepSing) scap = std::min<uint64_t>(smax, scap * 2);
		if (dbg()) fprintf(stderr, "sk count pass: entry buffers too small, retrying with %llu / %llu\n", (unsigned long long)wcap, (unsigned long long)scap);
	}
	time_end(h, KMR_TIME_COUNT, tca, tcb);
	return 0;
}
template <int W> int sk_append_early(kmr_handle *h, SkFinalize<W> &p) {
	FinalizeCounters &c = p.c; const FinalizeCounters &early_c = p.early_c; unsigned long long *cur = p.cur; const uint64_t early_slots = p.early_slots;
	const size_t eb = 8ull * (W + 1);
	if (cur[0] + early_slots > packed_entries(h, h->ue)) {
		DevBuf bigger;
		HIPCHK(h, bigger.alloc(eb * (cur[0] + early_slots + 4096)));
		HIPCHK(h, hipMemcpyAsync(bigger.get(), h->ue.get(), eb * cur[0], hipMemcpyDeviceToDevice, h->stream)); HIPCHK(h, hipStreamSynchronize(h->stream));
		h->ue = std::move(bigger);
	}
	HIPCHK(h, hipMemcpyAsync((uint8_t *)h->ue.get<uint64_t>() + eb * cur[0], h->early.ue.get<uint64_t>(), eb * early_slots, hipMemcpyDeviceToDevice, h->stream));
	cur[0] += early_slots;
	c.unique += early_c.unique; c.singletons += early_c.singletons; c.weak_kept += early_c.weak_kept; c.sing_kept += early_c.sing_kept;
	c.saturated += early_c.saturated; c.sat_sightings += early_c.sat_sightings;
	h->stats.unique_kmers = c.unique; h->stats.singleton_kmers = p.f.has_singletons ? c.singletons : 0;
	return 0;
}

template <int W> int finalize_superkmer_t(kmr_handle *h, uint32_t min_depth) {
	int rc = sync_state(h);
	if (rc) return rc;
	hipEvent_t ea, eb; time_begin(h, 1, &ea, &eb);
	SkFinalize<W> p;
	p.f = finalize_params(h, min_depth);
	p.keepSing = p.f.has_singletons && min_depth <= 1;
	p.ext = h->ext;
	p.tracking = h->cfg.size_tracker != 0;
	if (!h->l1.head) { rc = pool_reserve(h, h->l1, 0, false); if (rc) return rc; }
	rc = arena_reset(h); if (rc) return rc;
	p.nl = h->sk_state ? sk_list_count(h->sk_bits) : 1;
	if (h->sk_state) {
		hipLaunchKernelGGL(sk_close_kernel, dim3(grid_for(p.nl)), dim3(256), 0, h->stream, h->sk_state.get<unsigned long long>(), p.nl, h->l1.chunk_count.get<uint32_t>(), h->l1.cap);
		HIPCHK(h, hipGetLastError());
	}
	p.refined = h->sk_state && h->sk_fine_shift > 0;
	if (p.refined) { rc = sk_refine_lists(h, p.nl); if (rc) return rc; }
	rc = build_csr(h, h->l1, p.nl, 0, &p.ls, &p.lc, &p.nch); if (rc) return rc;
	rc = sk_entry_buffers<W>(h, p, h->stats.raw_good_kmers); if (rc) return rc;
	rc = sk_count_uniform<W>(h, p.tracking, p.uni, p.f.uni_wbits); if (rc) return rc;
	h->last_count_uniform = p.uni;
	if (p.tracking) { rc = sk_track_view(h, p.tv); if (rc) return rc; }
	p.lgMain = sk_own_lists<W>(h, p.refined);
	bool device_error = false;
	rc = sk_early_takeover<W>(h, p, min_depth, device_error); if (rc) return rc;
	if (device_error) { time_end(h, 1, ea, eb); return sync_state(h); }
	rc = sk_long_items<W>(h, p); if (rc) return rc;
	bool overflowed = false;
	rc = sk_count_pass<W>(h, p, overflowed); if (rc) return rc;
	if (overflowed) { time_end(h, 1, ea, eb); return fail(h, KMR_ERR_CAPACITY, "entry buffers of the count pass overflowed at their upper bound (internal sizing error)"); }
	h->stats.unique_kmers = p.c.unique;
	h->stats.singleton_kmers = p.f.has_singletons ? p.c.singletons : 0;
	if (p.tracking) { rc = sk_track_elements(h, p.tv, p.f.has_singletons); if (rc) return rc; }
	if (p.early_slots) { rc = sk_append_early<W>(h, p); if (rc) return rc; }
	h->early.active = false;
	hipEvent_t tma, tmb; time_begin(h, KMR_TIME_BUCKETS, &tma, &tmb);
	rc = finish_maps_from_entries(h, p.wc, p.sc, p.cur[0], p.cur[1], p.c.weak_kept, p.c.sing_kept, p.keepSing, !p.ext);
	time_end(h, KMR_TIME_BUCKETS, tma, tmb);
	if (rc) return rc;
	h->last_saturated_keys = 0; h->last_saturated_batches = 0;
	if (p.c.saturated) { rc = saturated_fix_t<W>(h, p.ls, p.lc, p.nl, p.c.saturated, p.c.sat_sightings, p.f.has_singletons); if (rc) return rc; }
	time_end(h, 1, ea, eb);
	h->has_singletons = p.keepSing;
	h->stats.weak_entries = h->weak.n; h->stats.singleton_entries = p.keepSing ? h->sing.n : 0;
	h->finalized = true; h->map_gen++;
	rc = sync_state(h);
	if (!rc && !h->arena_overflow.empty()) rc = arena_reset(h);
	return rc;
}
template <int W> int count_prefix_superkmer_t(kmr_handle *h, uint32_t min_depth, uint64_t hi) {
	int rc = sync_state(h); if (rc) return rc;
	FinalizeParams f = finalize_params(h, min_depth);
	const bool keepSing = f.has_singletons && min_depth <= 1;
	h->early.active = false;
	if (h->ext || h->cfg.size_tracker || keepSing || (h->sk_state && h->sk_fine_shift > 0) || !h->sk_state) return KMR_OK;
	const uint64_t nl = sk_list_count(h->sk_bits);
	if (hi > nl) hi = nl;
	if (hi == 0) return KMR_OK;
	rc = arena_reset(h); if (rc) return rc;
	hipLaunchKernelGGL(sk_close_kernel, dim3(grid_for(nl)), dim3(256), 0, h->stream, h->sk_state.get<unsigned long long>(), nl, h->l1.chunk_count.get<uint32_t>(), h->l1.cap);
	HIPCHK(h, hipGetLastError());
	uint64_t *ls = nullptr, *lc = nullptr; uint32_t nch = 0;
	rc = build_csr(h, h->l1, nl, 0, &ls, &lc, &nch); if (rc) return rc;
	const uint64_t G = h->stats.raw_good_kmers;
	const uint64_t slack = (uint64_t)num_cus(h) * 4 * 8192 + 16;
	uint64_t want = (uint64_t)((double)G * ((double)hi / (double)nl) / (f.has_singletons ? 6.0 : 2.5)) + slack;
	if (h->tune.early_entry_share >= 0) { want = (uint64_t)((double)G * h->tune.early_entry_share) + 16384; h->early.ue.reset(); }
	rc = h->early.ue.reserve(h, "early count ue", 8ull * (W + 1) * want); if (rc) return rc;
	rc = h->early.cursor.reserve(h, "early count cursor", 16); if (rc) return rc;
	rc = h->early.fc.reserve(h, "early count fc", sizeof(FinalizeCounters)); if (rc) return rc;
	rc = h->early.err.reserve(h, "early count error word", 4); if (rc) return rc;
	HIPCHK(h, hipMemsetAsync(h->early.cursor.get<unsigned long long>(), 0, 16, h->stream)); HIPCHK(h, hipMemsetAsync(h->early.fc.get(), 0, sizeof(FinalizeCounters), h->stream));
	HIPCHK(h, hipMemsetAsync(h->early.err.get<uint32_t>(), 0, 4, h->stream));
	bool uni = false;
	if (!h->peer_uni_mixed) { rc = sk_count_uniform<W>(h, false, uni, f.uni_wbits); if (rc) return rc; }
	const SkTrackView tv{};
	SkLong<W> lg = sk_own_lists<W>(h, false);
	lg.long_threshold = h->tune.long_list_chunks ? h->tune.long_list_chunks : 1024;
	uint32_t *sc = nullptr;
	rc = arena_get(h, &sc, h->nb_sing); if (rc) return rc;
	HIPCHK(h, hipMemsetAsync(sc, 0, 4 * h->nb_sing, h->stream));
	CountOut out{};
	out.wentries = h->early.ue.get<uint64_t>(); out.wcursor = h->early.cursor.get<unsigned long long>(); out.wcap = packed_entries(h, h->early.ue);
	out.scursor = h->early.cursor.get<unsigned long long>() + 1;
	out.singCount = sc; out.fc = (FinalizeCounters *)h->early.fc.get(); out.err = h->early.err.get<uint32_t>();
	rc = zero_work_counter(h); if (rc) return rc;
	const uint64_t n_work = hi > lg.list_first ? (hi - lg.list_first + lg.list_stride - 1) / lg.list_stride : 0;
	if (n_work) {
		const int grid = (int)std::min<uint64_t>((uint64_t)num_cus(h) * 4, (n_work + SK_LBATCH) / SK_LBATCH);
		SkCountLaunch<W> k;
		rc = sk_count_select<W>(h, false, false, uni, k); if (rc) return rc;
		hipEvent_t a, b; time_begin(h, KMR_TIME_COUNT, &a, &b);
		hipLaunchKernelGGL(k.kern, dim3(grid), dim3(SKC_THREADS), k.smem, h->stream, pool_view(h, h->l1), ls, lc, hi, h->k, out, f, h->work_counter.get<unsigned int>(), sk_dbg_flags("KMR_SK_COUNT_DBG"), tv, lg);
		time_end(h, KMR_TIME_COUNT, a, b);
		HIPCHK(h, hipGetLastError());
	}
	h->early.active = true; h->early.hi = hi; h->early.min_depth = min_depth;
	return KMR_OK;
}
int count_prefix_superkmer(kmr_handle *h, uint32_t min_depth, uint64_t hi) { return with_w(h, [&](auto W) { return count_prefix_superkmer_t<W()>(h, min_depth, hi); }); }
int finalize_superkmer(kmr_handle *h, uint32_t min_depth) { return with_w(h, [&](auto W) { return finalize_superkmer_t<W()>(h, min_depth); }); }

template <class M> void release(kmr_handle *h) { static_cast<M &>(*h) = M(); }

void free_partition_state(kmr_handle *h) {
	release<BuildMem>(h);
	if (h->tb_copy_stream) { hipStreamDestroy(h->tb_copy_stream); h->tb_copy_stream = nullptr; for (int a = 0; a < 2; a++) { hipEventDestroy(h->tb_ready[a]); hipEventDestroy(h->tb_consumed[a]); h->tb_set_used[a] = false; } }
}

}

extern "C" {

uint32_t kmr_abi_version(void) { return KMR_ABI_VERSION; }

int kmr_config_init(kmr_config *c) {
	if (!c) return KMR_ERR_INVALID_ARG;
	memset(c, 0, sizeof(*c));
	c->struct_size = sizeof(*c);
	c->value_kind = KMR_VALUE_COUNT_DIR; c->min_weight = 0.10f; c->min_quality_score = 3; c->fastq_start_char = 33;
	c->ext_min_quality = 20; c->separate_singletons = 1; c->kmer_subsample = 1; c->device = -1; c->rank = 0; c->world_size = 1;
	c->estimated_depth = 20.0; c->estimated_error_rate = 0.35; c->kmers_per_bucket = 32; c->num_parts = 1; c->part_idx = 0;
	return KMR_OK;
}

const char *kmr_last_error(const kmr_handle *h) { return h ? h->err.c_str() : g_create_error.c_str(); }

int kmr_create(const kmr_config *cfg, kmr_handle **out) {
	if (!cfg || !out) return fail(nullptr, KMR_ERR_INVALID_ARG, "null argument");
	*out = nullptr;
	if (cfg->struct_size != sizeof(kmr_config)) return fail(nullptr, KMR_ERR_INVALID_ARG, "kmr_config.struct_size mismatch (ABI)");
	if (cfg->k < 1 || cfg->k > 128) return fail(nullptr, KMR_ERR_INVALID_ARG, "k must be in 1..128");
	if (cfg->world_size < 1 || cfg->rank >= cfg->world_size) return fail(nullptr, KMR_ERR_INVALID_ARG, "bad rank/world_size");
	if (cfg->value_kind > KMR_VALUE_EXT) return fail(nullptr, KMR_ERR_INVALID_ARG, "bad value_kind");
	if (cfg->hash_kind > KMR_HASH_LOOKUP8) return fail(nullptr, KMR_ERR_INVALID_ARG, "bad hash_kind");
	int ndev = 0;
	if (hipGetDeviceCount(&ndev) != hipSuccess || ndev == 0) return fail(nullptr, KMR_ERR_NO_DEVICE, "no HIP device: this library has no CPU path");
	kmr_handle *h = new kmr_handle();
	h->cfg = *cfg;
	if (h->cfg.kmer_subsample == 0) h->cfg.kmer_subsample = 1;
	if (h->cfg.num_parts == 0) h->cfg.num_parts = 1;
	h->k = cfg->k; h->kb = (cfg->k + 3) / 4; h->W = (h->kb + 7) / 8; h->ext = cfg->value_kind == KMR_VALUE_EXT;
	h->hkb = h->kb | (cfg->hash_kind << 16);
	memset(&h->stats, 0, sizeof(h->stats));
	int rc = 0;
	do {
		if (cfg->device >= 0) { if (hipSetDevice(cfg->device) != hipSuccess) { rc = fail(nullptr, KMR_ERR_NO_DEVICE, "hipSetDevice failed"); break; } }
		if (hipGetDevice(&h->device) != hipSuccess) { rc = fail(nullptr, KMR_ERR_NO_DEVICE, "hipGetDevice failed"); break; }
		if (hipStreamCreate(&h->stream) != hipSuccess) { rc = fail(nullptr, KMR_ERR_HIP, "hipStreamCreate failed"); break; }
		uint64_t w = cfg->num_buckets_weak, s = cfg->num_buckets_singleton;
		const double depth = cfg->estimated_depth > 0 ? cfg->estimated_depth : 20.0;
		const uint32_t kpb = cfg->kmers_per_bucket ? cfg->kmers_per_bucket : 32;
		const uint64_t raw = cfg->estimated_raw_kmers / (cfg->world_size > 1 ? cfg->world_size : 1);
		if (w == 0) { unsigned long est = (unsigned long)(int)(raw / depth); w = est / kpb + 1; }
		if (s == 0) { unsigned long est = cfg->separate_singletons ? (unsigned long)(raw * cfg->estimated_error_rate) : 1; s = est / kpb + 1; }
		h->nb_weak = resize_buckets(w); h->nb_sing = resize_buckets(s);
		h->has_singletons = cfg->separate_singletons != 0;
		uint64_t want = cfg->max_table_entries ? (uint64_t)(cfg->max_table_entries / 0.7) : (uint64_t)(cfg->estimated_raw_kmers * 0.45 / 0.6);
		if (cfg->world_size > 1 && !cfg->max_table_entries) want /= cfg->world_size;
		uint32_t lg = 16; while ((1ull << lg) < want && lg < 40) lg++;
		h->log2cap = lg;
		double P[256]; quality_table(P, cfg->min_quality_score, cfg->fastq_start_char);
		if (h->dP.alloc(sizeof(P)) != hipSuccess || h->dstats.alloc(sizeof(DevStats)) != hipSuccess || h->derr.alloc(4) != hipSuccess) { rc = fail(nullptr, KMR_ERR_OOM, "hipMalloc failed"); break; }
		hipMemcpy(h->dP.get<double>(), P, sizeof(P), hipMemcpyHostToDevice); hipMemset(h->dstats.get<DevStats>(), 0, sizeof(DevStats)); hipMemset(h->derr.get<uint32_t>(), 0, 4);
		if (cfg->build_mode > 3) { rc = fail(nullptr, KMR_ERR_INVALID_ARG, "bad build_mode"); break; }
		h->partition_mode = cfg->build_mode != 1;
		uint32_t wish_w = 0, wish_m = 0, wish_o = 0;
		const bool sk_auto = cfg->build_mode == 0 && cfg->world_size <= 1 && sk_geometry(h->k, 0, wish_w, wish_m, wish_o);
		h->auto_mode = cfg->build_mode == 0;
		const bool sk_ready = sk_geometry(h->k, 0, wish_w, wish_m, wish_o);
		if (cfg->build_mode == 3 || sk_auto || sk_ready) {
			if (!sk_geometry(h->k, 0, h->sk_win, h->sk_m, h->sk_off)) { rc = fail(nullptr, KMR_ERR_UNSUPPORTED, "build_mode 3 (super-k-mer lists) needs k >= 13"); break; }
			h->superkmer_mode = cfg->build_mode == 3 || sk_auto;
			double Pk[256];
			for (int cidx = 0; cidx < 256; cidx++) { double wv = 1.0; for (uint32_t jj = 0; jj < h->k; jj++) wv *= P[cidx]; Pk[cidx] = wv; }
			memcpy(h->hPk, Pk, sizeof(Pk)); memcpy(h->hP, P, sizeof(h->hP));
			if (h->dPk.alloc(2 * sizeof(Pk)) != hipSuccess) { rc = fail(nullptr, KMR_ERR_OOM, "hipMalloc failed"); break; }
			hipMemcpy(h->dPk.get<double>(), Pk, sizeof(Pk), hipMemcpyHostToDevice);
			double Rp[256]; bool fast = true;
			for (int cidx = 0; cidx < 256; cidx++) Rp[cidx] = P[cidx] != 0.0 ? 1.0 / P[cidx] : 0.0;
			for (int a = 0; a < 256 && fast; a++) for (int b = 0; b < 256; b++) {
				if (P[a] == 0.0 || P[b] == 0.0) continue;
				const double q0 = P[a] * Rp[b];
				if (std::fma(std::fma(-q0, P[b], P[a]), Rp[b], q0) != P[a] / P[b]) { fast = false; break; }
			}
			h->sk_fast_div = fast;
			hipMemcpy(h->dPk.get<double>() + 256, Rp, sizeof(Rp), hipMemcpyHostToDevice);
		}
		if (cfg->size_tracker && (!h->superkmer_mode || h->ext || cfg->world_size > 1)) { rc = fail(nullptr, KMR_ERR_UNSUPPORTED, "size_tracker: kept by the super-k-mer build (build_mode 0 / 3, direction-counting values, k >= 13) of a single partition"); break; }
		if (!h->partition_mode) {
			rc = alloc_table(h, h->log2cap, h->slots, h->extslots);
			if (rc) { g_create_error = h->err; break; }
		}
		if (hipStreamSynchronize(h->stream) != hipSuccess) { rc = fail(nullptr, KMR_ERR_HIP, std::string("table clear failed: ") + hipGetErrorString(hipGetLastError())); break; }
	} while (0);
	if (rc) { kmr_destroy(h); return rc; }
	*out = h;
	return KMR_OK;
}

static void exchange_destroy_comm(kmr_handle *h);
void kmr_destroy(kmr_handle *h) {
	if (!h) return;
	if (h->stream) hipStreamSynchronize(h->stream);
	for (int which = 0; which < KMR_TIME_GROUPS; which++) for (auto &pr : h->pending_events[which]) { hipEventDestroy(pr.first); hipEventDestroy(pr.second); }
	release<HandleMem>(h);
	free_partition_state(h);
	exchange_destroy_comm(h);
	release<ExchangeMem>(h);
	if (h->stream) hipStreamDestroy(h->stream);
	delete h;
}

int kmr_num_buckets(const kmr_handle *h, int which, uint64_t *out) {
	if (!h || !out) return KMR_ERR_INVALID_ARG;
	if (which == KMR_MAP_WEAK) *out = h->finalized && h->weak.present ? h->weak.nb : h->nb_weak;
	else if (which == KMR_MAP_SINGLETON) *out = h->finalized && h->sing.present ? h->sing.nb : h->nb_sing;
	else return KMR_ERR_UNSUPPORTED;
	return KMR_OK;
}

int kmr_reset(kmr_handle *h) {
	if (!h) return KMR_ERR_INVALID_ARG;
	hipSetDevice(h->device);
	HIPCHK(h, hipStreamSynchronize(h->stream));
	clear_map(h->weak); clear_map(h->sing);
	int rc = 0;
	if (h->partition_mode) {
		if (h->l1.head) HIPCHK(h, hipMemsetAsync(h->l1.head.get<unsigned int>(), 0, 4, h->stream));
		h->l1.used_ub = 0;
		h->inserted_records = 0;
		h->qual_mixed = false;
		h->sk_uni_w = SK_UNI_NONE; h->sk_uni_mixed = false; h->peer_uni_w = SK_UNI_NONE; h->peer_uni_mixed = false; h->peers_declare = false;
		h->xr_lo = 0; h->xr_hi = ~0ull; h->early.active = false;
		if (h->d_uni) { const uint32_t init[2] = {SK_UNI_NONE, 0u}; HIPCHK(h, hipMemcpyAsync(h->d_uni.get<uint32_t>(), init, 8, hipMemcpyHostToDevice, h->stream)); HIPCHK(h, hipStreamSynchronize(h->stream)); }
		if (h->sk_state) hipLaunchKernelGGL(sk_state_init_kernel, dim3(grid_for(sk_list_count(h->sk_bits))), dim3(256), 0, h->stream, h->sk_state.get<unsigned long long>(), sk_list_count(h->sk_bits));
		if (h->l1_state) {
			hipLaunchKernelGGL(partition_state_init_kernel, dim3(partition_blocks(h)), dim3(256), 0, h->stream, h->l1_state.get<uint8_t>(),
			                   h->l1_state.cap() / (size_t)partition_blocks(h), h->bits1, (uint32_t)partition_blocks(h));
			h->l1_state_dirty = false;
		}
	} else {
		if (!h->slots) rc = alloc_table(h, h->log2cap, h->slots, h->extslots);
		else rc = clear_table_any(h, h->slots.get(), h->extslots.get<ExtSlot>(), h->log2cap);
		if (rc) return rc;
	}
	HIPCHK(h, hipMemsetAsync(h->dstats.get<DevStats>(), 0, sizeof(DevStats), h->stream));
	HIPCHK(h, hipMemsetAsync(h->derr.get<uint32_t>(), 0, 4, h->stream));
	memset(&h->stats, 0, sizeof(h->stats));
	h->occupied = h->pending_kmers = 0; h->stream_base = 0; h->reads = 0; h->subtracted = 0; h->xc_job_bases = 0; h->xc_bytes_to_peers = 0;
	h->trk_n = 0; h->trk_elems.clear();
	h->trk_next = 128; h->trk_raw = h->trk_good = 0; h->trk_bounds.clear(); h->trk_snap_raw.clear(); h->trk_snap_good.clear();
	h->finalized = false; h->map_gen++; h->has_singletons = h->cfg.separate_singletons != 0;
	return KMR_OK;
}
int kmr_release_table(kmr_handle *h) {
	if (!h) return KMR_ERR_INVALID_ARG;
	if (!h->finalized) return fail(h, KMR_ERR_STATE, "kmr_release_table before kmr_finalize");
	hipSetDevice(h->device);
	h->slots.reset(); h->extslots.reset();
	if (h->partition_mode) free_partition_state(h);
	return KMR_OK;
}

void *kmr_stream(kmr_handle *h) { return h ? (void *)h->stream : nullptr; }

int kmr_set_stream_origin(kmr_handle *h, uint64_t ordinal) {
	if (!h) return KMR_ERR_INVALID_ARG;
	if (h->finalized) return fail(h, KMR_ERR_STATE, "kmr_set_stream_origin after kmr_finalize");
	if (ordinal > MAX_STREAM_ORDINAL) return fail(h, KMR_ERR_CAPACITY, "stream ordinals have 40 bits");
	h->stream_base = ordinal;
	return KMR_OK;
}

int kmr_tune(kmr_handle *h, const char *knob, double value) {
	if (!h || !knob) return KMR_ERR_INVALID_ARG;
	const std::string k(knob);
	if (k == "target_list_records") h->tune.target_list = value >= 1 ? (uint64_t)value : 2048;
	else if (k == "sub_batch_bases") h->tune.sub_batch_bases = value >= 1 ? (uint64_t)value : 0;
	else if (k == "recycle_chunks") h->tune.recycle = value < 0 ? -1 : (value != 0 ? 1 : 0);
	else if (k == "partition_blocks") h->tune.part_blocks = value >= 1 ? (int)value : 0;
	else if (k == "entry_share") h->tune.entry_share = value;
	else if (k == "early_entry_share") h->tune.early_entry_share = value;
	else if (k == "saturated_batch_bytes") h->tune.saturated_batch_bytes = value >= 1 ? (uint64_t)value : 0;
	else if (k == "lookup_table") h->tune.no_lut = value == 0;
	else if (k == "stream_lookups") h->tune.no_stream_lookups = value == 0;
	else if (k == "long_list_chunks") h->tune.long_list_chunks = value < 2 ? 2 : (uint64_t)value;
	else if (k == "lean_extract") h->tune.no_lean_extract = value == 0;
	else if (k == "uniform_count") h->tune.no_uniform_count = value == 0;
	else if (k == "packed_direct") h->tune.no_packed_direct = value == 0;
	else if (k == "pow2_lists") h->tune.pow2_lists = value != 0;
	else if (k == "list_aim") h->tune.list_aim = value >= 1 ? (uint64_t)value : 0;
	else if (k == "twobit_piece_bases") h->tune.twobit_piece_bases = (uint64_t)value;
	else if (k == "exchange_fail_once") h->tune.exchange_fail_once = value != 0;
	else if (k == "binned_buckets_min") h->tune.binned_min = value >= 0 ? (uint64_t)value : ~0ull;
	else if (k == "coarse_lists") h->tune.no_coarse_lists = value == 0;
	else if (k == "select_timing") h->tune.select_timing = value != 0;
	else if (k == "dump_timing") h->tune.dump_timing = value != 0;
	else if (k == "pairs_timing") h->tune.pairs_timing = value != 0;
	else if (k == "dedup_timing") h->tune.dedup_timing = value != 0;
	else if (k == "partition_units") h->tune.partition_units = value >= 1 && value <= 8192 ? (uint32_t)value : 0;
	else if (k == "pair_hash_bits") h->tune.pair_hash_bits = value >= 1 && value < 64 ? (uint32_t)value : 64;
	else if (k == "dump_piece_bytes") h->tune.dump_piece_bytes = value >= 1 ? (uint64_t)value : 0;
	else if (k == "narrow_tallies") h->tune.no_narrow = value == 0;
	else if (k == "keep_level1_state") h->tune.no_l1_state = value == 0;
	else if (k == "superkmer_window") {
		if (h->superkmer_mode && !h->sk_state) { uint32_t w, m, o; if (!sk_geometry(h->k, 0, w, m, o, (uint32_t)value)) return fail(h, KMR_ERR_INVALID_ARG, "no minimizer geometry under that window"); h->sk_win = w; h->sk_m = m; h->sk_off = o; }
	}
	else if (k == "superkmer_minimizer") {
		if (h->superkmer_mode && !h->sk_state) { uint32_t w, m, o; if (!sk_geometry(h->k, (uint32_t)value, w, m, o)) return fail(h, KMR_ERR_INVALID_ARG, "no minimizer geometry for that length"); h->sk_win = w; h->sk_m = m; h->sk_off = o; }
	}
	else return fail(h, KMR_ERR_INVALID_ARG, "unknown tuning knob '" + k + "'");
	return KMR_OK;
}

int kmr_build_info(kmr_handle *h, const char *what, double *value) {
	if (!h || !what || !value) return KMR_ERR_INVALID_ARG;
	const std::string k(what);
	if (k == "lists") *value = h->sk_state ? (double)sk_list_count(h->sk_bits) : 0.0;
	else if (k == "uniform_count") *value = h->last_count_uniform ? 1.0 : 0.0;
	else if (k == "chunk_pool_chunks") *value = (double)h->l1.cap;
	else if (k == "superkmer_window") *value = (double)h->sk_win;
	else if (k == "early_lists") *value = (double)h->last_early_hi;
	else if (k == "early_entries") *value = (double)h->last_early_entries;
	else if (k == "early_overflowed") *value = h->last_early_overflowed ? 1.0 : 0.0;
	else if (k == "saturated_keys") *value = (double)h->last_saturated_keys;
	else if (k == "saturated_batches") *value = (double)h->last_saturated_batches;
	else if (k == "device_blocks_live") *value = (double)g_blocks_live.load();
	else if (k == "filter_score_ms") *value = h->last_score_ms;
	else if (k == "select_ms") *value = h->last_select_ms;
	else if (k == "select_write_ms") *value = h->last_write_ms;
	else if (k == "pairs_ms") *value = h->last_pairs_ms;
	else if (k == "pairs_parse_ms") *value = h->last_pairs_parse_ms;
	else if (k == "pairs_sort_ms") *value = h->last_pairs_sort_ms;
	else if (k == "pair_hash_collisions") *value = (double)h->last_pair_hash_collisions;
	else if (k == "dedup_ms") *value = h->last_dedup_ms;
	else if (k == "dedup_key_ms") *value = h->last_dedup_key_ms;
	else if (k == "dedup_sort_ms") *value = h->last_dedup_sort_ms;
	else if (k == "dedup_consensus_ms") *value = h->last_dedup_consensus_ms;
	else if (k == "dump_size_ms") *value = h->last_dump_size_ms;
	else if (k == "dump_write_ms") *value = h->last_dump_write_ms;
	else return fail(h, KMR_ERR_INVALID_ARG, "unknown build figure '" + k + "'");
	return KMR_OK;
}

int kmr_sync(kmr_handle *h) { if (!h) return KMR_ERR_INVALID_ARG; hipSetDevice(h->device); return sync_state(h); }

int kmr_add_reads_dev(kmr_handle *h, const void *dev_bases, const void *dev_quals, const void *dev_offsets, uint64_t n_reads,
                      uint64_t total_bases, uint64_t first_global_read_idx, const void *dev_discarded) {
	if (!h) return KMR_ERR_INVALID_ARG;
	if (h->finalized) return fail(h, KMR_ERR_STATE, "kmr_add_reads after kmr_finalize");
	if (n_reads == 0) return KMR_OK;
	if (!dev_bases || !dev_offsets) return fail(h, KMR_ERR_INVALID_ARG, "null device buffer");
	hipSetDevice(h->device);
	const ReadsView rv = reads_view(dev_bases, dev_quals, dev_offsets, n_reads, dev_discarded, h->stream_base, first_global_read_idx);
	if (h->stream_base + total_bases > MAX_STREAM_ORDINAL) return fail(h, KMR_ERR_CAPACITY, "more than 2^40 input bases on one handle");
	if (h->partition_mode && !h->superkmer_mode && !h->ext && h->stream_base + total_bases > (1ull << 32))
		return fail(h, KMR_ERR_CAPACITY, "build_mode 2 orders occurrences by a 32-bit stream ordinal: at most 2^32 input bases per handle without extension values (use build_mode 0 / 3 or 1)");
	int rc = h->superkmer_mode ? add_reads_superkmer(h, rv, total_bases) : (h->partition_mode ? add_reads_partition(h, rv, total_bases) : add_reads_dev_any(h, rv, total_bases));
	h->stream_base += total_bases; h->reads += n_reads; h->stats.reads = h->reads;
	return rc;
}

static hipError_t tb_stage_copy(kmr_handle *h, int set, int which, const void *src, size_t bytes, void **dst) {
	DevBuf &buf = h->tb_stage[set][which];
	if (buf.cap() < bytes + 128) {
		if (buf) { hipError_t e0 = hipStreamSynchronize(h->stream); if (e0 != hipSuccess) return e0; }
		hipError_t e = buf.alloc(bytes + bytes / 8 + 4096); if (e != hipSuccess) return e;
	}
	*dst = buf.get();
	return bytes ? hipMemcpyAsync(buf.get(), src, bytes, hipMemcpyHostToDevice, h->tb_copy_stream) : hipSuccess;
}
static int tb_pipeline_ready(kmr_handle *h) {
	if (h->tb_copy_stream) return 0;
	HIPCHK(h, hipStreamCreateWithFlags(&h->tb_copy_stream, hipStreamNonBlocking));
	for (int i = 0; i < 2; i++) { HIPCHK(h, hipEventCreateWithFlags(&h->tb_ready[i], hipEventDisableTiming)); HIPCHK(h, hipEventCreateWithFlags(&h->tb_consumed[i], hipEventDisableTiming)); }
	return 0;
}

#define TBCHK(call) do { hipError_t e_ = (call); if (e_ != hipSuccess) { hipStreamSynchronize(h->tb_copy_stream); hipStreamSynchronize(h->stream); h->err = std::string(#call) + ": " + hip_err_text(e_); return e_ == hipErrorOutOfMemory ? KMR_ERR_OOM : KMR_ERR_HIP; } } while (0)
}
template <class Stage, class Feed> static int tb_feed_pieces(kmr_handle *h, const uint64_t *offsets, uint64_t n_reads, Stage &&stage, Feed &&feed) {
	{ int rcp = tb_pipeline_ready(h); if (rcp) return rcp; }
	const uint64_t piece_bases = h->tune.twobit_piece_bases ? h->tune.twobit_piece_bases : (1ull << 28);
	int rc = KMR_OK; int set = 0;
	h->call_bases_hint = n_reads ? offsets[n_reads] - offsets[0] : 0;
	struct HintReset { kmr_handle *h; ~HintReset() { h->call_bases_hint = 0; } } hint_reset{h};
	for (uint64_t r0 = 0; r0 < n_reads && rc == KMR_OK; set ^= 1) {
		uint64_t r1 = r0 + 1;
		while (r1 < n_reads && offsets[r1 + 1] - offsets[r0] <= piece_bases) r1++;
		if (h->tb_set_used[set]) TBCHK(hipStreamWaitEvent(h->tb_copy_stream, h->tb_consumed[set], 0));
		{ int rcs = stage(set, r0, r1); if (rcs) return rcs; }
		TBCHK(hipEventRecord(h->tb_ready[set], h->tb_copy_stream));
		TBCHK(hipStreamWaitEvent(h->stream, h->tb_ready[set], 0));
		rc = feed(r0, r1);
		TBCHK(hipEventRecord(h->tb_consumed[set], h->stream)); h->tb_set_used[set] = true;
		r0 = r1;
	}
	hipStreamSynchronize(h->tb_copy_stream);
	if (!rc) rc = sync_state(h);
	else hipStreamSynchronize(h->stream);
	return rc;
}
extern "C" {

int kmr_add_reads(kmr_handle *h, const char *bases, const char *quals, const uint64_t *offsets, uint64_t n_reads,
                  uint64_t first_global_read_idx, const uint8_t *discarded) {
	if (!h) return KMR_ERR_INVALID_ARG;
	if (h->finalized) return fail(h, KMR_ERR_STATE, "kmr_add_reads after kmr_finalize");
	if (n_reads == 0) return KMR_OK;
	if (!bases || !offsets) return fail(h, KMR_ERR_INVALID_ARG, "null buffer");
	hipSetDevice(h->device);
	void *db = nullptr, *dq = nullptr, *doff = nullptr, *dd = nullptr;
	auto stage = [&](int set, uint64_t r0, uint64_t r1) -> int {
		const uint64_t m = r1 - r0, total = offsets[r1] - offsets[r0];
		dq = nullptr; dd = nullptr;
		TBCHK(tb_stage_copy(h, set, 0, bases + offsets[r0], total, &db)); TBCHK(tb_stage_copy(h, set, 2, offsets + r0, 8 * (m + 1), &doff));
		if (quals) TBCHK(tb_stage_copy(h, set, 6, quals + offsets[r0], total, &dq));
		if (discarded) TBCHK(tb_stage_copy(h, set, 7, discarded + r0, m, &dd));
		TBCHK(hipMemsetAsync((uint8_t *)db + total, 0, 64, h->tb_copy_stream)); if (dq) TBCHK(hipMemsetAsync((uint8_t *)dq + total, 0, 64, h->tb_copy_stream));
		return KMR_OK;
	};
	auto feed = [&](uint64_t r0, uint64_t r1) {
		return kmr_add_reads_dev(h, (uint8_t *)db - offsets[r0], dq ? (uint8_t *)dq - offsets[r0] : nullptr, doff, r1 - r0, offsets[r1] - offsets[r0], first_global_read_idx + r0, dd);
	};
	return tb_feed_pieces(h, offsets, n_reads, stage, feed);
}

static bool sk_packed_direct_ok(kmr_handle *h, bool has_quals, int uniform_quality) {
	if (!h->superkmer_mode || h->ext || h->cfg.size_tracker || h->tune.no_lean_extract || h->tune.no_packed_direct || sp_debug_extract(h) || has_quals || h->qual_mixed) return false;
	const DevParams dp = dev_params(h);
	if (dp.subsample > 1 || dp.num_parts > 1 || (dp.sub_wnb | dp.sub_snb) != 0 || (dp.world > 1 && !h->sk_exchange)) return false;
	return uniform_quality == 0 || uniform_quality == 127 || h->hP[uniform_quality] > 0.0;
}
int kmr_add_reads_twobit_dev(kmr_handle *h, const void *dev_twobit, const void *dev_twobit_offsets, const void *dev_offsets,
                             const void *dev_markup_offsets, const void *dev_markup_pos, const void *dev_markup_char,
                             const void *dev_quals, int uniform_quality, uint64_t n_reads, uint64_t total_bases,
                             uint64_t first_global_read_idx, const void *dev_discarded) {
	if (!h) return KMR_ERR_INVALID_ARG;
	if (h->finalized) return fail(h, KMR_ERR_STATE, "kmr_add_reads after kmr_finalize");
	if (n_reads == 0) return KMR_OK;
	if (!dev_twobit || !dev_offsets) return fail(h, KMR_ERR_INVALID_ARG, "null device buffer");
	if (dev_markup_offsets && (!dev_markup_pos || !dev_markup_char)) return fail(h, KMR_ERR_INVALID_ARG, "markup offsets without markups");
	if (uniform_quality < 0 || uniform_quality > 255 || (dev_quals && uniform_quality)) return fail(h, KMR_ERR_INVALID_ARG, "uniform_quality: 0, or the one quality character of a batch without a quality array");
	hipSetDevice(h->device);
	const bool direct = sk_packed_direct_ok(h, dev_quals != nullptr, uniform_quality);
	if (!direct && h->tb_bases.cap() < total_bases + 64) {
		if (h->tb_bases) HIPCHK(h, hipStreamSynchronize(h->stream));
		HIPCHK(h, h->tb_bases.alloc(total_bases + 64));
		HIPCHK(h, hipMemsetAsync(h->tb_bases.get<uint8_t>(), 0, total_bases + 64, h->stream));
	}
	if (h->tb_len.cap() < 4 * (n_reads + 1)) {
		if (h->tb_len) HIPCHK(h, hipStreamSynchronize(h->stream));
		h->tb_rel.reset(); h->tb_off.reset(); h->tb_len.reset();
		HIPCHK(h, h->tb_rel.alloc(8 * (n_reads + 1))); HIPCHK(h, h->tb_off.alloc(8 * (n_reads + 1))); HIPCHK(h, h->tb_len.alloc(4 * (n_reads + 1)));
	}
	const uint64_t *tboff = (const uint64_t *)dev_twobit_offsets;
	if (!tboff) {
		int rc = twobit_byte_offsets(h, (const uint64_t *)dev_offsets, n_reads, h->tb_len.get<uint32_t>(), h->tb_off.get<uint64_t>()); if (rc) return rc;
		tboff = h->tb_off.get<uint64_t>();
	}
	if (direct) {
		{ int rc = twobit_rel_offsets(h, (const uint64_t *)dev_offsets, n_reads, h->tb_rel.get<uint64_t>()); if (rc) return rc; }
		if (h->stream_base + total_bases > MAX_STREAM_ORDINAL) return fail(h, KMR_ERR_CAPACITY, "more than 2^40 input bases on one handle");
		const ReadsView rv = reads_view(nullptr, nullptr, h->tb_rel.get<uint64_t>(), n_reads, dev_discarded, h->stream_base, first_global_read_idx);
		SkPacked pkd; pkd.bytes = (const uint8_t *)dev_twobit; pkd.off = tboff; pkd.mk_off = (const uint64_t *)dev_markup_offsets; pkd.mk_pos = (const uint32_t *)dev_markup_pos; pkd.mk_char = (const uint8_t *)dev_markup_char;
		h->packed_direct = &pkd; h->uniform_q_hint = uniform_quality ? uniform_quality : -1;
		const int rc = add_reads_superkmer(h, rv, total_bases);
		h->packed_direct = nullptr; h->uniform_q_hint = -1;
		h->stream_base += total_bases; h->reads += n_reads; h->stats.reads = h->reads;
		return rc;
	}
	{ int rc = twobit_unpack(h, (const uint8_t *)dev_twobit, tboff, (const uint64_t *)dev_offsets, (const uint64_t *)dev_markup_offsets, (const uint32_t *)dev_markup_pos,
	                         (const uint8_t *)dev_markup_char, n_reads, h->tb_bases.get<uint8_t>(), h->tb_rel.get<uint64_t>()); if (rc) return rc; }
	const void *q = dev_quals;
	if (!dev_quals && uniform_quality) {
		if (h->tb_quals.cap() < total_bases + 64) {
			if (h->tb_quals) HIPCHK(h, hipStreamSynchronize(h->stream));
// ... 800 lines not shown
```

### kmernator_amd/csrc/kmr_buckets.hpp

```cpp
#ifndef KMR_BUCKETS_HPP_
#define KMR_BUCKETS_HPP_

#include "kmr_partition.hpp"

namespace kmr {

int sort_pairs_u64_u32(void *tmp, size_t *tmp_bytes, const unsigned long long *keys_in, unsigned long long *keys_out, const unsigned int *vals_in, unsigned int *vals_out, size_t n, hipStream_t stream);

static const int BB_TILE = 8192;
static const int BB_THREADS = 512;
static const int BB_GROUP_THREADS = 256;
static const int BB_PER_THREAD = BB_TILE / BB_THREADS;
static const int BB_MAX_BITS = 10;
static const int BB_MAX_GROUP_BITS = 8;
static const uint32_t BB_GROUP_CAP = 1536;
template <int W> __host__ __device__ constexpr uint32_t bb_group_cap() { return W == 1 ? BB_GROUP_CAP : 1344u; }

__host__ __device__ __forceinline__ uint64_t bb_pack_value(uint32_t count, uint32_t weighted_bits, uint32_t dir) { return (uint64_t)(count | (dir << 16)) | ((uint64_t)weighted_bits << 32); }

struct BbInput {
	const uint64_t *entries;
	const uint64_t *seg_start;
	const uint32_t *seg_count;
	uint32_t n_seg;
	uint64_t n_slots;
	uint32_t holes;
};

template <int W> __device__ __forceinline__ void bb_load_entry(const uint64_t *entries, uint64_t e, uint64_t (&w)[W + 1]) {
	if constexpr (W == 1) { const uint4 v = ((const uint4 *)entries)[e]; w[0] = (uint64_t)v.x | ((uint64_t)v.y << 32); w[1] = (uint64_t)v.z | ((uint64_t)v.w << 32); }
	else {
#pragma unroll
		for (int q = 0; q <= W; q++) w[q] = entries[e * (W + 1) + q];
	}
}
template <int W> __device__ __forceinline__ void bb_store_entry(uint64_t *entries, uint64_t e, const uint64_t (&w)[W + 1]) {
	if constexpr (W == 1) ((uint4 *)entries)[e] = make_uint4((uint32_t)w[0], (uint32_t)(w[0] >> 32), (uint32_t)w[1], (uint32_t)(w[1] >> 32));
	else {
#pragma unroll
		for (int q = 0; q <= W; q++) entries[e * (W + 1) + q] = w[q];
	}
}

__device__ __forceinline__ uint32_t bb_segment_of(const BbInput &in, uint64_t s0) {
	if (!in.seg_start) return 0;
	uint32_t lo = 0, hi = in.n_seg;
	while (hi - lo > 1) { const uint32_t mid = (lo + hi) >> 1; if (in.seg_start[mid] <= s0) lo = mid; else hi = mid; }
	return lo;
}

template <int W>
__global__ __launch_bounds__(BB_THREADS)
void bb_hist_kernel(BbInput in, uint32_t shift, uint32_t bits, uint32_t kb, uint64_t nb, uint32_t tiles_per_block, uint32_t *hist) {
	__shared__ uint32_t lh[1 << BB_MAX_BITS];
	__shared__ uint32_t s_seg;
	const int t = threadIdx.x;
	const uint32_t bins = 1u << bits, mask = bins - 1;
	const uint64_t n_tiles = (in.n_slots + BB_TILE - 1) / BB_TILE;
	const uint64_t tile0 = (uint64_t)blockIdx.x * tiles_per_block;
	uint32_t curSeg = 0xffffffffu;
	for (uint32_t i = t; i < bins; i += BB_THREADS) lh[i] = 0;
	__syncthreads();
	for (uint64_t tile = tile0; tile < tile0 + tiles_per_block && tile < n_tiles; tile++) {
		const uint64_t s0 = tile * BB_TILE;
		if (t == 0) s_seg = bb_segment_of(in, s0);
		__syncthreads();
		const uint32_t seg = s_seg;
		if (seg != curSeg) {
			if (curSeg != 0xffffffffu) {
				for (uint32_t i = t; i < bins; i += BB_THREADS) { const uint32_t c = lh[i]; if (c) { atomicAdd(&hist[((uint64_t)curSeg << bits) + i], c); lh[i] = 0; } }
				__syncthreads();
			}
			curSeg = seg;
		}
		const uint64_t segEnd = in.seg_start ? in.seg_start[seg] + in.seg_count[seg] : in.n_slots;
#pragma unroll 4
		for (int i = 0; i < BB_PER_THREAD; i++) {
			const uint64_t e = s0 + (uint64_t)i * BB_THREADS + t;
			if (e >= segEnd) continue;
			uint64_t ew[W + 1];
			bb_load_entry<W>(in.entries, e, ew);
			if (in.holes && ew[W] == 0) continue;
			Key<W> key;
#pragma unroll
			for (int q = 0; q < W; q++) key.w[q] = ew[q];
			const uint64_t b = key_hash<W>(key, kb) & (nb - 1);
			atomicAdd(&lh[(uint32_t)(b >> shift) & mask], 1u);
		}
		__syncthreads();
	}
	if (curSeg != 0xffffffffu) for (uint32_t i = t; i < bins; i += BB_THREADS) { const uint32_t c = lh[i]; if (c) atomicAdd(&hist[((uint64_t)curSeg << bits) + i], c); }
}

#ifndef KMR_INSTANCE_TU
__global__ void bb_pad_kernel(const uint32_t *hist, uint64_t n, uint32_t *padded, unsigned int *max_count) {
	unsigned int m = 0;
	for (uint64_t i = blockIdx.x * (uint64_t)blockDim.x + threadIdx.x; i < n; i += (uint64_t)gridDim.x * blockDim.x) {
		const uint32_t c = hist[i];
		if (padded) padded[i] = (c + BB_TILE - 1) / BB_TILE * BB_TILE;
		m = c > m ? c : m;
	}
	for (int o = 32; o > 0; o >>= 1) { const unsigned int x = (unsigned int)__shfl_xor((int)m, o, 64); m = x > m ? x : m; }
	if ((threadIdx.x & 63) == 0 && m) atomicMax(max_count, m);
}
__global__ void bb_cursor_init_kernel(const uint64_t *start, uint64_t n, unsigned long long *cursor) {
	for (uint64_t i = blockIdx.x * (uint64_t)blockDim.x + threadIdx.x; i < n; i += (uint64_t)gridDim.x * blockDim.x) cursor[i] = start[i];
}
#endif

template <int W>
__global__ __launch_bounds__(BB_THREADS)
void bb_scatter_kernel(BbInput in, uint32_t shift, uint32_t bits, uint32_t kb, uint64_t nb, unsigned long long *cursor, uint64_t *out_entries) {
	__shared__ uint32_t lh[1 << BB_MAX_BITS];
	__shared__ unsigned long long lbase[1 << BB_MAX_BITS];
	__shared__ uint32_t s_seg;
	const int t = threadIdx.x;
	const uint32_t bins = 1u << bits, mask = bins - 1;
	const uint64_t n_tiles = (in.n_slots + BB_TILE - 1) / BB_TILE;
	for (uint64_t tile = blockIdx.x; tile < n_tiles; tile += gridDim.x) {
		const uint64_t s0 = tile * BB_TILE;
		__syncthreads();
		if (t == 0) s_seg = bb_segment_of(in, s0);
		for (uint32_t i = t; i < bins; i += BB_THREADS) lh[i] = 0;
		__syncthreads();
		const uint32_t seg = s_seg;
		const uint64_t segEnd = in.seg_start ? in.seg_start[seg] + in.seg_count[seg] : in.n_slots;
		uint32_t where[BB_PER_THREAD];
#pragma unroll
		for (int i = 0; i < BB_PER_THREAD; i++) {
			const uint64_t e = s0 + (uint64_t)i * BB_THREADS + t;
			where[i] = 0xffffffffu;
			if (e >= segEnd) continue;
			uint64_t ew[W + 1];
			bb_load_entry<W>(in.entries, e, ew);
			if (in.holes && ew[W] == 0) continue;
			Key<W> key;
#pragma unroll
			for (int q = 0; q < W; q++) key.w[q] = ew[q];
			const uint32_t bin = (uint32_t)((key_hash<W>(key, kb) & (nb - 1)) >> shift) & mask;
			where[i] = (bin << 16) | atomicAdd(&lh[bin], 1u);
		}
		__syncthreads();
		for (uint32_t i = t; i < bins; i += BB_THREADS) { const uint32_t c = lh[i]; if (c) lbase[i] = atomicAdd(&cursor[((uint64_t)seg << bits) + i], (unsigned long long)c); }
		__syncthreads();
#pragma unroll
		for (int i = 0; i < BB_PER_THREAD; i++) {
			if (where[i] == 0xffffffffu) continue;
			const uint64_t e = s0 + (uint64_t)i * BB_THREADS + t;
			uint64_t ew[W + 1];
			bb_load_entry<W>(in.entries, e, ew);
			bb_store_entry<W>(out_entries, lbase[where[i] >> 16] + (where[i] & 0xffffu), ew);
		}
	}
}

static const int BB_GROUP_PER_THREAD = (BB_GROUP_CAP + BB_GROUP_THREADS - 1) / BB_GROUP_THREADS;
template <int W> __host__ __device__ constexpr size_t bb_group_smem_bytes() { return (size_t)bb_group_cap<W>() * (8 * W + 8 + 2 + 2); }

template <int W>
__global__ __launch_bounds__(BB_GROUP_THREADS, W <= 2 ? 4 : 1)
void bb_group_kernel(const uint64_t *entries, uint64_t *keys, uint32_t *vals, const uint64_t *gstart, const uint32_t *gcount, uint64_t n_groups, uint32_t gbits, uint32_t kb, uint64_t nb,
                     uint64_t *start, uint64_t n_total, uint32_t *err) {
	extern __shared__ __attribute__((aligned(16))) uint8_t gsm[];
	uint64_t *skeys = (uint64_t *)gsm;
	constexpr uint32_t CAP = bb_group_cap<W>();
	uint64_t *svalw = skeys + (size_t)CAP * W;
	uint16_t *sbucket = (uint16_t *)(svalw + CAP);
	uint16_t *final_ = sbucket + CAP;
	__shared__ uint32_t bcnt[1 << BB_MAX_GROUP_BITS], bstart[(1 << BB_MAX_GROUP_BITS) + 1], bscan[BB_GROUP_THREADS / 64];
	const int t = threadIdx.x;
	const uint32_t nbk = 1u << gbits;
	for (uint64_t G = blockIdx.x; G < n_groups; G += gridDim.x) {
		const uint64_t base = gstart[G];
		const uint32_t n = gcount[G];
		__syncthreads();
		if ((uint32_t)t < nbk) bcnt[t] = 0;
		if (n > CAP) { if (t == 0) atomicOr(err, (uint32_t)ERR_ENTRIES_FULL); continue; }
		__syncthreads();
		uint64_t ew[BB_GROUP_PER_THREAD][W + 1]; uint32_t lb[BB_GROUP_PER_THREAD];
#pragma unroll
		for (int u = 0; u < BB_GROUP_PER_THREAD; u++) {
			const uint32_t i = (uint32_t)u * BB_GROUP_THREADS + t;
			lb[u] = 0xffffffffu;
			if (i < n) bb_load_entry<W>(entries, base + i, ew[u]);
		}
#pragma unroll
		for (int u = 0; u < BB_GROUP_PER_THREAD; u++) {
			const uint32_t i = (uint32_t)u * BB_GROUP_THREADS + t;
			if (i >= n) continue;
			Key<W> key;
#pragma unroll
			for (int q = 0; q < W; q++) key.w[q] = ew[u][q];
			lb[u] = (uint32_t)(key_hash<W>(key, kb) & (nb - 1)) & (nbk - 1);
			atomicAdd(&bcnt[lb[u]], 1u);
		}
		__syncthreads();
		{
			const uint32_t c = (uint32_t)t < nbk ? bcnt[t] : 0u;
			uint32_t incl = c;
#pragma unroll
			for (int o = 1; o < 64; o <<= 1) { const uint32_t x = (uint32_t)__shfl_up((int)incl, o, 64); if ((t & 63) >= o) incl += x; }
			if ((t & 63) == 63) bscan[t >> 6] = incl;
			__syncthreads();
			uint32_t before = 0;
			for (int w = 0; w < (t >> 6); w++) before += bscan[w];
			if ((uint32_t)t < nbk) { bstart[t] = before + incl - c; start[G * nbk + t] = base + before + incl - c; bcnt[t] = 0; }
			if (t == 0) { bstart[nbk] = n; if (G == n_groups - 1) start[nb] = n_total; }
		}
		__syncthreads();
#pragma unroll
		for (int u = 0; u < BB_GROUP_PER_THREAD; u++) {
			if (lb[u] == 0xffffffffu) continue;
			const uint32_t pos = bstart[lb[u]] + atomicAdd(&bcnt[lb[u]], 1u);
#pragma unroll
			for (int q = 0; q < W; q++) skeys[(size_t)pos * W + q] = ew[u][q];
			svalw[pos] = ew[u][W];
			sbucket[pos] = (uint16_t)lb[u];
		}
		__syncthreads();
		for (uint32_t p = t; p < n; p += BB_GROUP_THREADS) {
			const uint32_t b = sbucket[p];
			const uint32_t s = bstart[b], e = bstart[b + 1];
			Key<W> mine;
#pragma unroll
			for (int q = 0; q < W; q++) mine.w[q] = skeys[(size_t)p * W + q];
			uint32_t rank = 0;
#pragma unroll 4
			for (uint32_t qx = s; qx < e; qx++) {
				Key<W> other;
#pragma unroll
				for (int q = 0; q < W; q++) other.w[q] = skeys[(size_t)qx * W + q];
				rank += (key_lt<W>(other, mine) || (key_eq<W>(other, mine) && qx < p)) ? 1u : 0u;
			}
			final_[s + rank] = (uint16_t)p;
		}
		__syncthreads();
		for (uint32_t p = t; p < n; p += BB_GROUP_THREADS) {
			const uint32_t i = final_[p];
#pragma unroll
			for (int q = 0; q < W; q++) keys[(base + p) * W + q] = skeys[(size_t)i * W + q];
			const uint64_t vw_ = svalw[i];
			vals[(base + p) * 3] = (uint32_t)vw_ & 0xffffu; vals[(base + p) * 3 + 1] = (uint32_t)(vw_ >> 32); vals[(base + p) * 3 + 2] = ((uint32_t)vw_ >> 16) & 0xffffu;
		}
	}
}

template <int W>
__global__ __launch_bounds__(256)
void bb_unpack_kernel(const uint64_t *entries, uint64_t n_slots, uint32_t kb, uint64_t nb, uint64_t *keys, uint32_t *vals, uint32_t *counts) {
	for (uint64_t e = blockIdx.x * (uint64_t)blockDim.x + threadIdx.x; e < n_slots; e += (uint64_t)gridDim.x * blockDim.x) {
		uint64_t ew[W + 1];
		bb_load_entry<W>(entries, e, ew);
		Key<W> key;
#pragma unroll
		for (int q = 0; q < W; q++) { key.w[q] = ew[q]; keys[e * W + q] = ew[q]; }
		vals[e * 3] = (uint32_t)ew[W] & 0xffffu; vals[e * 3 + 1] = (uint32_t)(ew[W] >> 32); vals[e * 3 + 2] = ((uint32_t)ew[W] >> 16) & 0xffffu;
		if (ew[W] != 0) atomicAdd(&counts[key_hash<W>(key, kb) & (nb - 1)], 1u);
	}
}

}
#endif
```

### kmernator_amd/csrc/kmr_host.hpp

```cpp
#ifndef KMR_HOST_HPP_
#define KMR_HOST_HPP_

#include <hip/hip_runtime.h>
#include <unistd.h>

#include <algorithm>
#include <atomic>
#include <cstdio>
#include <memory>
#include <string>
#include <type_traits>
#include <utility>
#include <vector>

#include "../../include/kmernator_amd.h"

#define KMR_HIDDEN __attribute__((visibility("hidden")))

namespace kmr { struct SkPacked; }

namespace kmr_host KMR_HIDDEN {

inline std::string g_create_error;

inline thread_local char g_oom_note[160] = "";
inline std::atomic<long long> g_blocks_live{0};
inline hipError_t dev_malloc(void **p, size_t bytes) {
	hipError_t e = hipMalloc(p, bytes);
	if (e == hipSuccess) { if (*p) g_blocks_live++; return e; }
	if (e != hipErrorOutOfMemory) return e;
	size_t fr = 0, tot = 0;
	for (int attempt = 0; attempt < 6; attempt++) {
		(void)hipGetLastError();
		hipDeviceSynchronize();
		if (hipMemGetInfo(&fr, &tot) != hipSuccess || bytes > tot) break;
		usleep(20000u << attempt);
		e = hipMalloc(p, bytes);
		if (e == hipSuccess && *p) g_blocks_live++;
		if (e != hipErrorOutOfMemory) return e;
	}
	(void)hipGetLastError();
	hipMemGetInfo(&fr, &tot);
	snprintf(g_oom_note, sizeof(g_oom_note), " [requested %.3f GB; device has %.3f GB free of %.3f GB]", bytes / 1e9, fr / 1e9, tot / 1e9);
	*p = nullptr;
	return hipErrorOutOfMemory;
}

class DevBuf {
public:
	DevBuf() = default;
	DevBuf(DevBuf &&o) noexcept : p_(o.p_), cap_(o.cap_) { o.p_ = nullptr; o.cap_ = 0; }
	DevBuf &operator=(DevBuf &&o) noexcept { if (this != &o) { reset(); std::swap(p_, o.p_); std::swap(cap_, o.cap_); } return *this; }
	~DevBuf() { reset(); }
	void reset() { if (p_) { hipFree(p_); g_blocks_live--; } p_ = nullptr; cap_ = 0; }
	hipError_t alloc(size_t bytes) {
		reset();
		void *p = nullptr;
		const hipError_t e = dev_malloc(&p, bytes);
		if (e == hipSuccess) { p_ = p; cap_ = bytes; }
		return e;
	}
	int reserve(kmr_handle *h, const char *what, size_t need, size_t bytes = 0);
	template <class T = void> T *get() const { return (T *)p_; }
	size_t cap() const { return cap_; }
	explicit operator bool() const { return p_ != nullptr; }
private:
	void *p_ = nullptr;
	size_t cap_ = 0;
};

struct DevMap {
	uint64_t nb = 0, n = 0;
	DevBuf start;
	DevBuf keys;
	DevBuf vals;
	DevBuf sweight;
	DevBuf spkt;
	DevBuf image;
	bool present = false;
};

struct HostPool {
	DevBuf base, chunk_list, chunk_count, head;
	uint32_t cap = 0; size_t chunk_bytes = 0;
	uint64_t used_ub = 0;
	uint64_t presize = 0;
};

struct HandleMem {
	DevBuf slots, extslots;
	DevBuf dP, dstats, derr;
	DevMap weak, sing;
	DevBuf ix_start, ix_keys, ix_counts;
	DevBuf scratch_stats;
	DevBuf adopt_buf;
	DevBuf trk;
	DevBuf scan_sums;
	DevBuf score_buf;
	DevBuf lut;
	DevBuf dPk;
	DevBuf d_uni;
	DevBuf qrange;
	DevBuf sk_fine_state;
	struct Early { bool active = false; uint64_t hi = 0; uint32_t min_depth = 0; DevBuf ue, cursor, fc, err; } early;
	DevBuf dedup_tab;
	DevBuf xo_dev;
};
struct BuildMem {
	DevBuf sk_state;
	HostPool l1;
	DevBuf work_counter;
	DevBuf l1_state; bool l1_state_dirty = false;
	DevBuf arena; size_t arena_used = 0, arena_want = 0; std::vector<DevBuf> arena_overflow;
	DevBuf linear;
	DevBuf tile_count, kcap, koff;
	DevBuf ucnt, ufirst, u_start, u_end, u_read, umax;
	DevBuf tb_bases, tb_quals, tb_rel, tb_off, tb_len;
	uint64_t tb_quals_filled = 0; int tb_quals_char = -1;
	DevBuf tb_stage[2][8];
	DevBuf uw_keys, uw_vals, us_keys, us_b8, us_pkt;
	DevBuf ue, ue2;
};
struct ExchangeMem {
	DevBuf xc_small, xc_dcounts;
	DevBuf xc_send, xc_send2, xc_recv, xc_recv2;
};

}
using namespace kmr_host;

struct KMR_HIDDEN Tuning {
	uint64_t target_list = 2048;
	uint64_t sub_batch_bases = 0;
	int recycle = -1;
	int part_blocks = 0;
	double entry_share = -1.0;
	double early_entry_share = -1.0;
	uint64_t saturated_batch_bytes = 0;
	bool no_lut = false, no_narrow = false, no_l1_state = false, no_stream_lookups = false;
	uint64_t long_list_chunks = 0;
	uint64_t binned_min = 1ull << 18;
	uint64_t twobit_piece_bases = 0;
	uint64_t list_aim = 0;
	bool pow2_lists = false;
	bool no_packed_direct = false;
	bool no_uniform_count = false;
	bool no_lean_extract = false;
	bool exchange_fail_once = false;
	uint64_t dump_piece_bytes = 0;
	bool dump_timing = false;
	bool select_timing = false;
	bool pairs_timing = false;
	bool dedup_timing = false;
	uint32_t partition_units = 0;
	uint32_t pair_hash_bits = 64;
	bool no_coarse_lists = true;
};

struct KMR_HIDDEN kmr_handle : HandleMem, BuildMem, ExchangeMem {
	kmr_config cfg;
	Tuning tune;
	uint32_t k = 0, kb = 0, hkb = 0, W = 0;
	bool ext = false;
	int device = 0, ncu = 0;
	hipStream_t stream = nullptr;
	std::string err;
	uint32_t log2cap = 0;
	uint64_t occupied = 0;
	uint64_t pending_kmers = 0;
	uint64_t stream_base = 0, reads = 0;
	uint64_t nb_weak = 0, nb_sing = 0;
	bool finalized = false, has_singletons = true;
	kmr_handle *subtract = nullptr;
	uint64_t subtracted = 0;
	kmr_stats stats;
	bool partition_mode = false;
	bool superkmer_mode = false;
	uint64_t ix_lists = 0, ix_gen = ~0ull;
	uint64_t trk_n = 0; std::vector<uint64_t> trk_elems;
	long trk_next = 128; uint64_t trk_raw = 0, trk_good = 0; std::vector<unsigned long long> trk_bounds; std::vector<uint64_t> trk_snap_raw, trk_snap_good;
	bool sk_fast_div = false;
	bool sender_launch = false;
	bool sk_exchange = false;
	bool auto_mode = false;
	int bits1 = 0;
	uint64_t inserted_records = 0;
	uint64_t call_bases_hint = 0;
	uint32_t lut_log2 = 0;
	uint64_t lut_gen = ~0ull, map_gen = 0;
	hipStream_t tb_copy_stream = nullptr; hipEvent_t tb_ready[2] = {nullptr, nullptr}, tb_consumed[2] = {nullptr, nullptr}; bool tb_set_used[2] = {false, false};
	const kmr::SkPacked *packed_direct = nullptr;
	int uniform_q_hint = -1;
	uint32_t sk_bits = 0, sk_m = 0, sk_off = 0, sk_win = 0;
	double hP[256], hPk[256];
	uint32_t sk_uni_w = 0xffffffffu; bool sk_uni_mixed = false; bool last_count_uniform = false;
	uint32_t peer_uni_w = 0xffffffffu; bool peer_uni_mixed = false, peers_declare = false;
	uint64_t xr_lo = 0, xr_hi = ~0ull;
	uint64_t last_early_hi = 0, last_early_entries = 0;
	bool last_early_overflowed = false;
	double last_score_ms = 0, last_select_ms = 0, last_write_ms = 0;
	double last_dump_size_ms = 0, last_dump_write_ms = 0;
	double last_pairs_ms = 0, last_pairs_parse_ms = 0, last_pairs_sort_ms = 0;
	double last_dedup_ms = 0, last_dedup_key_ms = 0, last_dedup_sort_ms = 0, last_dedup_consensus_ms = 0;
	uint64_t last_pair_hash_collisions = 0;
	uint64_t last_saturated_keys = 0, last_saturated_batches = 0;
	bool qual_mixed = false;
	uint32_t sk_fine_shift = 0;
	uint32_t sk_min_override = 0;
	uint64_t xo_segcap = 0; std::vector<uint64_t> xo_counts; const void *xo_batch = nullptr; uint64_t xo_first = 0;
	void *xc_comm = nullptr; kmr_transport xc_tr = {nullptr, nullptr, nullptr};
	uint64_t xc_job_bases = 0, xc_bytes_to_peers = 0;
	hipEvent_t ev0 = nullptr, ev1 = nullptr;
	double ms[KMR_TIME_GROUPS] = {0};
	uint64_t launches[KMR_TIME_GROUPS] = {0};
	std::vector<std::pair<hipEvent_t, hipEvent_t> > pending_events[KMR_TIME_GROUPS];
};

struct OnDevice { int device = 0; };

struct KMR_HIDDEN kmr_picks : OnDevice {
	DevBuf text, picked;
	uint64_t n = 0, n_picked = 0, bytes = 0;
	DevBuf read_seg;
	std::vector<uint64_t> seg_table;
	uint32_t n_rounds = 1, n_inputs = 1;
	float round_depth[33] = {};
	uint8_t round_is_remainder[33] = {};
};

struct KMR_HIDDEN kmr_pairs : OnDevice {
	DevBuf mate, read1, read2;
	uint64_t n = 0, n_pairs = 0, n_full = 0, n_seq = 0, n_conflicts = 0;
};

struct KMR_HIDDEN kmr_text : OnDevice {
	DevBuf text;
	uint64_t kept = 0, bytes = 0;
};

struct KMR_HIDDEN kmr_reads : OnDevice {
	DevBuf bases, quals;
	DevBuf offsets;
	DevBuf name_off, name_len;
	uint64_t n = 0, total = 0, filtered = 0;
	uint32_t input_base = 0;
};

struct KMR_HIDDEN kmr_dedup : OnDevice {
	DevBuf disc, group_first, group_size, names;
	kmr_reads *cons = nullptr;
	~kmr_dedup() { delete cons; }
	uint64_t n = 0, n_groups = 0, affected = 0, name_bytes = 0;
	uint64_t skipped[4] = {0, 0, 0, 0};
};

namespace kmr_host KMR_HIDDEN {

inline std::string oom_note() { std::string s(g_oom_note); g_oom_note[0] = 0; return s; }

inline std::string hip_err_text(hipError_t e) { return std::string(hipGetErrorString(e)) + (e == hipErrorOutOfMemory ? oom_note() : std::string()); }

#define HIPCHK(h, call) do { hipError_t e_ = (call); if (e_ != hipSuccess) { \
	(h)->err = std::string(#call) + ": " + hip_err_text(e_); \
	return e_ == hipErrorOutOfMemory ? KMR_ERR_OOM : KMR_ERR_HIP; } } while (0)

inline int DevBuf::reserve(kmr_handle *h, const char *what, size_t need, size_t bytes) {
	if (p_ && cap_ >= need) return 0;
	if (!bytes) bytes = need;
	hipError_t e = p_ ? hipStreamSynchronize(h->stream) : hipSuccess;
	if (e == hipSuccess) e = alloc(bytes);
	if (e == hipSuccess) return 0;
	h->err = std::string("device buffer ") + what + " (" + std::to_string(bytes) + " bytes): " + hip_err_text(e);
	return e == hipErrorOutOfMemory ? KMR_ERR_OOM : KMR_ERR_HIP;
}

inline int fail(kmr_handle *h, int code, const std::string &msg) { const std::string m = code == KMR_ERR_OOM ? msg + oom_note() : msg; if (h) h->err = m; else g_create_error = m; return code; }

template <int N> using int_c = std::integral_constant<int, N>;
template <class F> auto with_w(const kmr_handle *h, F &&f) {
	switch (h->W) { case 1: return f(int_c<1>()); case 2: return f(int_c<2>()); case 3: return f(int_c<3>()); default: return f(int_c<4>()); }
}
template <class F> auto with_w_ext(const kmr_handle *h, F &&f) {
	return with_w(h, [&](auto W) { return h->ext ? f(W, std::true_type()) : f(W, std::false_type()); });
}

inline int grid_for(uint64_t n, int block = 256, int maxBlocks = 256 * 16) {
	uint64_t g = (n + block - 1) / block;
	if (g < 1) g = 1;
	if (g > (uint64_t)maxBlocks) g = maxBlocks;
	return (int)g;
}

template <class T> hipError_t alloc_n(DevBuf &b, T **p, size_t n) { const hipError_t e = b.alloc(std::max<size_t>(sizeof(T) * n, 256)); *p = b.get<T>(); return e; }

template <int N> struct EventTimer {
	hipEvent_t ev[N] = {}; bool on;
	explicit EventTimer(bool enabled) : on(enabled) { if (on) for (auto &e : ev) if (hipEventCreate(&e) != hipSuccess) { e = nullptr; on = false; } }
	~EventTimer() { for (auto e : ev) if (e) hipEventDestroy(e); }
	void mark(int i, hipStream_t s) { if (on) hipEventRecord(ev[i], s); }
	double ms(int a, int b) const { float t = 0; return on && hipEventElapsedTime(&t, ev[a], ev[b]) == hipSuccess ? t : 0.0; }
};

uint64_t resize_buckets(uint64_t n);
void quality_table(double P[256], unsigned minQ, unsigned startChar);
int exclusive_scan(kmr_handle *h, const uint32_t *in, uint64_t n, uint64_t *out );
int num_cus(kmr_handle *h);
struct ScoreDev { uint32_t *trim_offset, *trim_length; float *score; uint8_t *was_trimmed; };
int score_reads_core(kmr_handle *h, const uint8_t *s_b, const uint64_t *s_o, uint64_t n_reads, double minimum_kmer_score, int scoring_type,
                     uint32_t *trim_offset, uint32_t *trim_length, float *score, uint8_t *was_trimmed, ScoreDev *keep = nullptr);

int twobit_byte_offsets(kmr_handle *h, const uint64_t *offsets, uint64_t n, uint32_t *len, uint64_t *off);
int twobit_rel_offsets(kmr_handle *h, const uint64_t *offsets, uint64_t n, uint64_t *rel);
int twobit_unpack(kmr_handle *h, const uint8_t *twobit, const uint64_t *twobit_off, const uint64_t *offsets, const uint64_t *mk_off, const uint32_t *mk_pos, const uint8_t *mk_char,
                  uint64_t n, uint8_t *bases, uint64_t *rel);

}

namespace kmr {
int sort_pairs_u64_u32(void *tmp, size_t *tmp_bytes, const unsigned long long *keys_in, unsigned long long *keys_out, const unsigned int *vals_in, unsigned int *vals_out, size_t n, hipStream_t stream);
}

#endif
```

Before: 55.59 billion.

## Scatter bucket entries into fixed-capacity bins to skip histogram passes and syncs

Adds a fixed-stride radix scatter path for the weak-map bucket build. Each bin gets a capacity sized from the mean plus a slack term, so the histogram kernels, the host readback of the max bin and the stream syncs between passes are all skipped. The group kernel reads entries by stride. An overflow flag is checked once at the end, and if any bin overflowed, the count pass and bucket build are rerun with measured bins. This trades a larger scratch footprint and a rare full redo for fewer host round-trips and kernel launches.

Result: faster. 57.71 billion, median of 6 (+3.8%).

```diff
diff --git a/kmernator_amd/csrc/kmr_api.hip b/kmernator_amd/csrc/kmr_api.hip
--- a/kmernator_amd/csrc/kmr_api.hip
+++ b/kmernator_amd/csrc/kmr_api.hip
@@ -260,7 +260,7 @@
 
 }
 namespace kmr_host {
-int exclusive_scan(kmr_handle *h, const uint32_t *in, uint64_t n, uint64_t *out ) {
+int exclusive_scan_queue(kmr_handle *h, const uint32_t *in, uint64_t n, uint64_t *out ) {
 	const uint64_t nblocks = (n + SCAN_ITEMS - 1) / SCAN_ITEMS;
 	const size_t eb = sizeof(unsigned long long);
 	int rc = h->scan_sums.reserve(h, "scan_sums", eb * (nblocks + 1), eb * std::max<uint64_t>(nblocks + 1, 4096)); if (rc) return rc;
@@ -269,6 +269,10 @@
 	hipLaunchKernelGGL(scan_sums_kernel, dim3(1), dim3(256), 0, h->stream, sums, nblocks, total);
 	hipLaunchKernelGGL(scan_apply_kernel, dim3((unsigned)nblocks), dim3(256), 0, h->stream, in, n, sums, out);
 	HIPCHK(h, hipGetLastError());
+	return 0;
+}
+int exclusive_scan(kmr_handle *h, const uint32_t *in, uint64_t n, uint64_t *out ) {
+	const int rc = exclusive_scan_queue(h, in, n, out); if (rc) return rc;
 	HIPCHK(h, hipStreamSynchronize(h->stream));
 	return 0;
 }
@@ -773,7 +777,7 @@
 	return 0;
 }
 
-int finish_maps_from_entries(kmr_handle *h, uint32_t *wc, uint32_t *sc, uint64_t wslots, uint64_t sslots, uint64_t wn, uint64_t sn, bool keepSing, bool weak_uncounted = false);
+int finish_maps_from_entries(kmr_handle *h, uint32_t *wc, uint32_t *sc, uint64_t wslots, uint64_t sslots, uint64_t wn, uint64_t sn, bool keepSing, bool weak_uncounted = false, bool fixed_bins = false);
 CountOut count_out(kmr_handle *h, bool packed, unsigned long long *cursors, uint32_t *wc, uint32_t *sc, FinalizeCounters *fc);
 
 template <int W, bool EXT, int LOG2S, bool NARROW = false> int launch_count(kmr_handle *h, int grid, const uint64_t *ls, const uint64_t *lc, uint64_t nl, const CountOut &out, const FinalizeParams &f, int list_filter) {
@@ -962,8 +966,13 @@
 	return rc;
 }
 
-template <int W> int binned_buckets_t(kmr_handle *h, uint64_t wslots, uint64_t wn, bool &done) {
-	done = false;
+uint64_t bb_fixed_limit(uint64_t n, uint64_t bins, double scale) {
+	const double mean = (double)n / (double)bins;
+	return (n - 1) / bins + (uint64_t)(std::max(scale, 0.0) * (6.0 * std::sqrt(mean) + mean / 64.0 + 16.0));
+}
+
+template <int W> int binned_buckets_t(kmr_handle *h, uint64_t wslots, uint64_t wn, bool fixed_bins, bool &done) {
+	done = false; h->bb_overflow = nullptr;
 	DevMap &wm = h->weak;
 	const uint64_t nb = wm.nb;
 	uint32_t B = 0; while ((1ull << (B + 1)) <= nb) B++;
@@ -974,29 +983,62 @@
 	const uint32_t bits1 = R <= (uint32_t)BB_MAX_BITS ? R : (R + 1) / 2, bits2 = R - bits1;
 	const uint64_t bins1 = 1ull << bits1, groups = 1ull << R;
 	uint32_t *hist1 = nullptr, *hist2 = nullptr, *pad1 = nullptr; uint64_t *start1 = nullptr, *gstart = nullptr; unsigned long long *cursor = nullptr; unsigned int *dmax = nullptr;
-	int rc = arena_get(h, &hist1, bins1); if (rc) return rc;
+	int rc = 0;
+	BbInput in1; in1.entries = h->ue.get<uint64_t>(); in1.seg_start = nullptr; in1.seg_count = nullptr; in1.n_seg = 1; in1.n_slots = wslots; in1.holes = 1; in1.seg_stride = 0;
+	auto scatter_grid = [&](uint64_t n_slots) { const uint64_t tiles = (n_slots + BB_TILE - 1) / BB_TILE; return (unsigned)std::min<uint64_t>(tiles, (uint64_t)num_cus(h) * 8); };
+	auto scratch = [&](uint64_t entries) { return h->ue2.reserve(h, "ue2", 8ull * (W + 1) * entries); };
+	auto map_arrays = [&]() -> int {
+		int rc2 = wm.keys.reserve(h, "weak map keys", std::max<uint64_t>(8ull * W * wn, 8)); if (rc2) return rc2;
+		return wm.vals.reserve(h, "weak map vals", std::max<uint64_t>(12ull * wn, 8));
+	};
+	auto group_launch = [&](const uint64_t *entries, const uint64_t *gs, const uint32_t *gc, uint64_t in_stride, const uint32_t *overflow) -> int {
+		auto gk = bb_group_kernel<W>;
+		HIPCHK(h, hipFuncSetAttribute((const void *)gk, hipFuncAttributeMaxDynamicSharedMemorySize, (int)bb_group_smem_bytes<W>()));
+		int per_cu = 0;
+		if (hipOccupancyMaxActiveBlocksPerMultiprocessor(&per_cu, (const void *)gk, BB_GROUP_THREADS, bb_group_smem_bytes<W>()) != hipSuccess || per_cu < 1) per_cu = 4;
+		if (dbg()) fprintf(stderr, "bb_group<W=%d>: %d blocks per CU, %llu groups\n", W, per_cu, (unsigned long long)groups);
+		hipLaunchKernelGGL(gk, dim3((unsigned)std::min<uint64_t>(groups, (uint64_t)num_cus(h) * per_cu)), dim3(BB_GROUP_THREADS), bb_group_smem_bytes<W>(), h->stream, entries, wm.keys.get<uint64_t>(), wm.vals.get<uint32_t>(), gs, gc, groups, g, h->hkb, nb, wm.start.get<uint64_t>(), wn, h->derr.get<uint32_t>(), in_stride, overflow);
+		HIPCHK(h, hipGetLastError());
+		return 0;
+	};
+	const uint32_t shift1 = B - bits1, shift2 = g;
+	const uint64_t lim2 = std::min<uint64_t>(bb_fixed_limit(wn, groups, h->tune.bb_slack_groups), bb_group_cap<W>()), stride2 = std::max<uint64_t>(lim2, 1);
+	const uint64_t lim1 = bits2 ? bb_fixed_limit(wn, bins1, h->tune.bb_slack_bins) : 0, stride1 = std::max<uint64_t>((lim1 + BB_TILE - 1) / BB_TILE, 1) * BB_TILE;
+	if (fixed_bins && lim1 < (1ull << 32) && (!bits2 || groups * stride2 <= packed_entries(h, h->ue))) {
+		uint32_t *fill = nullptr, *overflow = nullptr;
+		rc = scratch(bits2 ? bins1 * stride1 : groups * stride2); if (rc) return rc;
+		rc = map_arrays(); if (rc) return rc;
+		rc = arena_get(h, &fill, bits2 ? bins1 + groups : groups); if (rc) return rc;
+		rc = arena_get(h, &gstart, groups + 1); if (rc) return rc;
+		rc = arena_get(h, &overflow, 1); if (rc) return rc;
+		HIPCHK(h, hipMemsetAsync(fill, 0, 4 * (bits2 ? bins1 + groups : groups), h->stream)); HIPCHK(h, hipMemsetAsync(overflow, 0, 4, h->stream));
+		auto scatter = [&](const BbInput &in, uint32_t shift, uint32_t bits, uint32_t *f, uint64_t limit, uint64_t stride, uint64_t *out) {
+			const unsigned grid = scatter_grid(in.n_slots);
+			if (W == 1 && !h->tune.bb_reload) hipLaunchKernelGGL((bb_scatter_fixed_kernel<W, W == 1>), dim3(grid), dim3(BB_THREADS), 0, h->stream, in, shift, bits, h->hkb, nb, f, (uint32_t)limit, stride, out, overflow);
+			else hipLaunchKernelGGL((bb_scatter_fixed_kernel<W, false>), dim3(grid), dim3(BB_THREADS), 0, h->stream, in, shift, bits, h->hkb, nb, f, (uint32_t)limit, stride, out, overflow);
+		};
+		uint32_t *gfill = fill;
+		if (!bits2) scatter(in1, shift1, bits1, fill, lim2, stride2, h->ue2.get<uint64_t>());
+		else {
+			scatter(in1, shift1, bits1, fill, lim1, stride1, h->ue2.get<uint64_t>());
+			BbInput in2; in2.entries = h->ue2.get<uint64_t>(); in2.seg_start = nullptr; in2.seg_count = fill; in2.n_seg = (uint32_t)bins1; in2.n_slots = bins1 * stride1; in2.holes = 0; in2.seg_stride = stride1;
+			gfill = fill + bins1;
+			scatter(in2, shift2, bits2, gfill, lim2, stride2, h->ue.get<uint64_t>());
+		}
+		HIPCHK(h, hipGetLastError());
+		rc = exclusive_scan_queue(h, gfill, groups, gstart); if (rc) return rc;
+		rc = group_launch(bits2 ? h->ue.get<uint64_t>() : h->ue2.get<uint64_t>(), gstart, gfill, stride2, overflow); if (rc) return rc;
+		h->bb_overflow = overflow; h->last_bb_path = 2;
+		done = true;
+		return 0;
+	}
+	rc = arena_get(h, &hist1, bins1); if (rc) return rc;
 	rc = arena_get(h, &start1, bins1 + 1); if (rc) return rc;
 	rc = arena_get(h, &cursor, groups); if (rc) return rc;
 	rc = arena_get(h, &dmax, 1); if (rc) return rc;
 	if (bits2) { rc = arena_get(h, &hist2, groups); if (rc) return rc; rc = arena_get(h, &pad1, bins1); if (rc) return rc; rc = arena_get(h, &gstart, groups + 1); if (rc) return rc; }
 	HIPCHK(h, hipMemsetAsync(hist1, 0, 4 * bins1, h->stream)); HIPCHK(h, hipMemsetAsync(dmax, 0, 4, h->stream));
-	BbInput in1; in1.entries = h->ue.get<uint64_t>(); in1.seg_start = nullptr; in1.seg_count = nullptr; in1.n_seg = 1; in1.n_slots = wslots; in1.holes = 1;
 	auto hist_grid = [&](uint64_t n_slots, uint32_t &tpb) { const uint64_t tiles = (n_slots + BB_TILE - 1) / BB_TILE; tpb = (uint32_t)std::max<uint64_t>(1, (tiles + 2047) / 2048); return (unsigned)((tiles + tpb - 1) / tpb); };
-	auto scatter_grid = [&](uint64_t n_slots) { const uint64_t tiles = (n_slots + BB_TILE - 1) / BB_TILE; return (unsigned)std::min<uint64_t>(tiles, (uint64_t)num_cus(h) * 8); };
-	auto scratch = [&](uint64_t entries) { return h->ue2.reserve(h, "ue2", 8ull * (W + 1) * entries); };
-	auto group_launch = [&](const uint64_t *entries, const uint64_t *gs, const uint32_t *gc) -> int {
-		int rc2 = wm.keys.reserve(h, "weak map keys", std::max<uint64_t>(8ull * W * wn, 8)); if (rc2) return rc2;
-		rc2 = wm.vals.reserve(h, "weak map vals", std::max<uint64_t>(12ull * wn, 8)); if (rc2) return rc2;
-		auto gk = bb_group_kernel<W>;
-		HIPCHK(h, hipFuncSetAttribute((const void *)gk, hipFuncAttributeMaxDynamicSharedMemorySize, (int)bb_group_smem_bytes<W>()));
-		int per_cu = 0;
-		if (hipOccupancyMaxActiveBlocksPerMultiprocessor(&per_cu, (const void *)gk, BB_GROUP_THREADS, bb_group_smem_bytes<W>()) != hipSuccess || per_cu < 1) per_cu = 4;
-		if (dbg()) fprintf(stderr, "bb_group<W=%d>: %d blocks per CU, %llu groups\n", W, per_cu, (unsigned long long)groups);
-		hipLaunchKernelGGL(gk, dim3((unsigned)std::min<uint64_t>(groups, (uint64_t)num_cus(h) * per_cu)), dim3(BB_GROUP_THREADS), bb_group_smem_bytes<W>(), h->stream, entries, wm.keys.get<uint64_t>(), wm.vals.get<uint32_t>(), gs, gc, groups, g, h->hkb, nb, wm.start.get<uint64_t>(), wn, h->derr.get<uint32_t>());
-		HIPCHK(h, hipGetLastError());
-		return 0;
-	};
-	const uint32_t shift1 = B - bits1;
 	uint32_t tpb = 1; unsigned grid = hist_grid(wslots, tpb);
 	hipLaunchKernelGGL(bb_hist_kernel<W>, dim3(grid), dim3(BB_THREADS), 0, h->stream, in1, shift1, bits1, h->hkb, nb, tpb, hist1);
 	unsigned int mx = 0;
@@ -1008,7 +1050,9 @@
 		rc = scratch(wn); if (rc) return rc;
 		hipLaunchKernelGGL(bb_cursor_init_kernel, dim3(grid_for(bins1)), dim3(256), 0, h->stream, (const uint64_t *)start1, bins1, cursor);
 		hipLaunchKernelGGL(bb_scatter_kernel<W>, dim3(scatter_grid(wslots)), dim3(BB_THREADS), 0, h->stream, in1, shift1, bits1, h->hkb, nb, cursor, h->ue2.get<uint64_t>());
-		rc = group_launch(h->ue2.get<uint64_t>(), start1, hist1); if (rc) return rc;
+		rc = map_arrays(); if (rc) return rc;
+		rc = group_launch(h->ue2.get<uint64_t>(), start1, hist1, 0, nullptr); if (rc) return rc;
+		h->last_bb_path = 1;
 		done = true;
 		return 0;
 	}
@@ -1019,8 +1063,7 @@
 	rc = scratch(std::max(padded_total, wn)); if (rc) return rc;
 	hipLaunchKernelGGL(bb_cursor_init_kernel, dim3(grid_for(bins1)), dim3(256), 0, h->stream, (const uint64_t *)start1, bins1, cursor);
 	hipLaunchKernelGGL(bb_scatter_kernel<W>, dim3(scatter_grid(wslots)), dim3(BB_THREADS), 0, h->stream, in1, shift1, bits1, h->hkb, nb, cursor, h->ue2.get<uint64_t>());
-	BbInput in2; in2.entries = h->ue2.get<uint64_t>(); in2.seg_start = start1; in2.seg_count = hist1; in2.n_seg = (uint32_t)bins1; in2.n_slots = padded_total; in2.holes = 0;
-	const uint32_t shift2 = g;
+	BbInput in2; in2.entries = h->ue2.get<uint64_t>(); in2.seg_start = start1; in2.seg_count = hist1; in2.n_seg = (uint32_t)bins1; in2.n_slots = padded_total; in2.holes = 0; in2.seg_stride = 0;
 	HIPCHK(h, hipMemsetAsync(hist2, 0, 4 * groups, h->stream)); HIPCHK(h, hipMemsetAsync(dmax, 0, 4, h->stream));
 	grid = hist_grid(padded_total, tpb);
 	hipLaunchKernelGGL(bb_hist_kernel<W>, dim3(grid), dim3(BB_THREADS), 0, h->stream, in2, shift2, bits2, h->hkb, nb, tpb, hist2);
@@ -1030,12 +1073,14 @@
 	if (mx > bb_group_cap<W>() || packed_entries(h, h->ue) < wn) return 0;
 	hipLaunchKernelGGL(bb_cursor_init_kernel, dim3(grid_for(groups)), dim3(256), 0, h->stream, (const uint64_t *)gstart, groups, cursor);
 	hipLaunchKernelGGL(bb_scatter_kernel<W>, dim3(scatter_grid(padded_total)), dim3(BB_THREADS), 0, h->stream, in2, shift2, bits2, h->hkb, nb, cursor, h->ue.get<uint64_t>());
-	rc = group_launch(h->ue.get<uint64_t>(), gstart, hist2); if (rc) return rc;
+	rc = map_arrays(); if (rc) return rc;
+	rc = group_launch(h->ue.get<uint64_t>(), gstart, hist2, 0, nullptr); if (rc) return rc;
+	h->last_bb_path = 1;
 	done = true;
 	return 0;
 }
 
-template <int W> int finish_maps_t(kmr_handle *h, uint32_t *wc, uint32_t *sc, uint64_t wslots, uint64_t sslots, uint64_t wn, uint64_t sn, bool keepSing, bool weak_uncounted) {
+template <int W> int finish_maps_t(kmr_handle *h, uint32_t *wc, uint32_t *sc, uint64_t wslots, uint64_t sslots, uint64_t wn, uint64_t sn, bool keepSing, bool weak_uncounted, bool fixed_bins) {
 	const uint32_t vw = h->ext ? 15 : 3;
 	DevMap &wm = h->weak, &sm = h->sing;
 	clear_map(wm); clear_map(sm);
@@ -1044,8 +1089,9 @@
 	int rc = wm.start.reserve(h, "weak map start", 8 * (wm.nb + 1)); if (rc) return rc;
 	rc = sm.start.reserve(h, "singleton map start", 8 * (sm.nb + 1)); if (rc) return rc;
 	bool weakDone = false;
+	h->last_bb_path = 0; h->bb_overflow = nullptr;
 	if (weak_uncounted) {
-		rc = binned_buckets_t<W>(h, wslots, wn, weakDone); if (rc) return rc;
+		rc = binned_buckets_t<W>(h, wslots, wn, fixed_bins, weakDone); if (rc) return rc;
 		if (!weakDone) {
 			if (key_entries(h, h->uw_keys) < wslots || !h->uw_vals) {
 				h->uw_keys.reset(); h->uw_vals.reset();
@@ -1058,7 +1104,7 @@
 		}
 	}
 	if (!weakDone) { rc = exclusive_scan(h, wc, wm.nb, wm.start.get<uint64_t>()); if (rc) return rc; }
-	if (keepSing) { rc = exclusive_scan(h, sc, sm.nb, sm.start.get<uint64_t>()); if (rc) return rc; }
+	if (keepSing) { rc = h->bb_overflow ? exclusive_scan_queue(h, sc, sm.nb, sm.start.get<uint64_t>()) : exclusive_scan(h, sc, sm.nb, sm.start.get<uint64_t>()); if (rc) return rc; }
 	else HIPCHK(h, hipMemsetAsync(sm.start.get<uint64_t>(), 0, 8 * (sm.nb + 1), h->stream));
 	if (!weakDone) {
 		rc = wm.keys.reserve(h, "weak map keys", std::max<uint64_t>(8ull * W * wm.n, 8)); if (rc) return rc;
@@ -1090,11 +1136,11 @@
 		hipLaunchKernelGGL((sort_buckets_kernel<W, 0>), dim3(grid_for(sm.nb, 4, 1 << 20)), dim3(256), 0, h->stream, ss, sm.start.get<uint64_t>(), sm.nb);
 	}
 	HIPCHK(h, hipGetLastError());
-	HIPCHK(h, hipStreamSynchronize(h->stream));
-	return 0;
-}
-int finish_maps_from_entries(kmr_handle *h, uint32_t *wc, uint32_t *sc, uint64_t wslots, uint64_t sslots, uint64_t wn, uint64_t sn, bool keepSing, bool weak_uncounted) {
-	return with_w(h, [&](auto W) { return finish_maps_t<W()>(h, wc, sc, wslots, sslots, wn, sn, keepSing, weak_uncounted); });
+	if (!h->bb_overflow) HIPCHK(h, hipStreamSynchronize(h->stream));
+	return 0;
+}
+int finish_maps_from_entries(kmr_handle *h, uint32_t *wc, uint32_t *sc, uint64_t wslots, uint64_t sslots, uint64_t wn, uint64_t sn, bool keepSing, bool weak_uncounted, bool fixed_bins) {
+	return with_w(h, [&](auto W) { return finish_maps_t<W()>(h, wc, sc, wslots, sslots, wn, sn, keepSing, weak_uncounted, fixed_bins); });
 }
 int finalize_partition(kmr_handle *h, uint32_t min_depth) { return with_w_ext(h, [&](auto W, auto EXT) { return finalize_partition_t<W(), EXT()>(h, min_depth); }); }
 template <int W, bool EXT> int insert_records_partition_t(kmr_handle *h, const void *recs, uint64_t n) {
@@ -1677,9 +1723,26 @@
 	if (p.early_slots) { rc = sk_append_early<W>(h, p); if (rc) return rc; }
 	h->early.active = false;
 	hipEvent_t tma, tmb; time_begin(h, KMR_TIME_BUCKETS, &tma, &tmb);
-	rc = finish_maps_from_entries(h, p.wc, p.sc, p.cur[0], p.cur[1], p.c.weak_kept, p.c.sing_kept, p.keepSing, !p.ext);
+	rc = finish_maps_from_entries(h, p.wc, p.sc, p.cur[0], p.cur[1], p.c.weak_kept, p.c.sing_kept, p.keepSing, !p.ext, h->tune.bb_fixed_bins);
 	time_end(h, KMR_TIME_BUCKETS, tma, tmb);
 	if (rc) return rc;
+	h->last_bb_fallback = false;
+	if (h->bb_overflow) {
+		uint32_t ovf = 0;
+		HIPCHK(h, hipMemcpyAsync(&ovf, h->bb_overflow, 4, hipMemcpyDeviceToHost, h->stream)); HIPCHK(h, hipStreamSynchronize(h->stream));
+		h->bb_overflow = nullptr;
+		if (ovf) {
+			if (dbg()) fprintf(stderr, "bucket build: a bin of the radix partition overflowed its capacity, again with measured bins\n");
+			h->last_bb_fallback = true;
+			rc = sk_count_pass<W>(h, p, overflowed); if (rc) return rc;
+			if (overflowed) { time_end(h, 1, ea, eb); return fail(h, KMR_ERR_CAPACITY, "entry buffers of the count pass overflowed at their upper bound (internal sizing error)"); }
+			if (p.early_slots) { rc = sk_append_early<W>(h, p); if (rc) return rc; }
+			time_begin(h, KMR_TIME_BUCKETS, &tma, &tmb);
+			rc = finish_maps_from_entries(h, p.wc, p.sc, p.cur[0], p.cur[1], p.c.weak_kept, p.c.sing_kept, p.keepSing, !p.ext, false);
+			time_end(h, KMR_TIME_BUCKETS, tma, tmb);
+			if (rc) return rc;
+		}
+	}
 	h->last_saturated_keys = 0; h->last_saturated_batches = 0;
 	if (p.c.saturated) { rc = saturated_fix_t<W>(h, p.ls, p.lc, p.nl, p.c.saturated, p.c.sat_sightings, p.f.has_singletons); if (rc) return rc; }
 	time_end(h, 1, ea, eb);
@@ -1936,6 +1999,10 @@
 	else if (k == "twobit_piece_bases") h->tune.twobit_piece_bases = (uint64_t)value;
 	else if (k == "exchange_fail_once") h->tune.exchange_fail_once = value != 0;
 	else if (k == "binned_buckets_min") h->tune.binned_min = value >= 0 ? (uint64_t)value : ~0ull;
+	else if (k == "bb_fixed_bins") h->tune.bb_fixed_bins = value != 0;
+	else if (k == "bb_slack_bins") h->tune.bb_slack_bins = value;
+	else if (k == "bb_slack_groups") h->tune.bb_slack_groups = value;
+	else if (k == "bb_reload") h->tune.bb_reload = value != 0;
 	else if (k == "coarse_lists") h->tune.no_coarse_lists = value == 0;
 	else if (k == "select_timing") h->tune.select_timing = value != 0;
 	else if (k == "dump_timing") h->tune.dump_timing = value != 0;
@@ -1966,6 +2033,8 @@
 	else if (k == "early_lists") *value = (double)h->last_early_hi;
 	else if (k == "early_entries") *value = (double)h->last_early_entries;
 	else if (k == "early_overflowed") *value = h->last_early_overflowed ? 1.0 : 0.0;
+	else if (k == "bb_path") *value = (double)h->last_bb_path;
+	else if (k == "bb_fallback") *value = h->last_bb_fallback ? 1.0 : 0.0;
 	else if (k == "saturated_keys") *value = (double)h->last_saturated_keys;
 	else if (k == "saturated_batches") *value = (double)h->last_saturated_batches;
 	else if (k == "device_blocks_live") *value = (double)g_blocks_live.load();
diff --git a/kmernator_amd/csrc/kmr_buckets.hpp b/kmernator_amd/csrc/kmr_buckets.hpp
--- a/kmernator_amd/csrc/kmr_buckets.hpp
+++ b/kmernator_amd/csrc/kmr_buckets.hpp
@@ -25,6 +25,7 @@
 	uint32_t n_seg;
 	uint64_t n_slots;
 	uint32_t holes;
+	uint64_t seg_stride;
 };
 
 template <int W> __device__ __forceinline__ void bb_load_entry(const uint64_t *entries, uint64_t e, uint64_t (&w)[W + 1]) {
@@ -154,13 +155,76 @@
 	}
 }
 
+template <int W, bool KEEP>
+__global__ __launch_bounds__(BB_THREADS)
+void bb_scatter_fixed_kernel(BbInput in, uint32_t shift, uint32_t bits, uint32_t kb, uint64_t nb, uint32_t *fill, uint32_t limit, uint64_t stride, uint64_t *out_entries, uint32_t *overflow) {
+	__shared__ uint32_t lh[1 << BB_MAX_BITS];
+	__shared__ unsigned long long lbase[1 << BB_MAX_BITS];
+	if (__syncthreads_or((int)*overflow)) return;
+	const int t = threadIdx.x;
+	const uint32_t bins = 1u << bits, mask = bins - 1;
+	const uint64_t n_tiles = (in.n_slots + BB_TILE - 1) / BB_TILE;
+	for (uint64_t tile = blockIdx.x; tile < n_tiles; tile += gridDim.x) {
+		const uint64_t s0 = tile * BB_TILE;
+		const uint64_t seg = in.seg_stride ? s0 / in.seg_stride : 0;
+		const uint64_t segEnd = in.seg_stride ? seg * in.seg_stride + (in.seg_count[seg] < in.seg_stride ? in.seg_count[seg] : in.seg_stride) : in.n_slots;
+		if (s0 >= segEnd) continue;
+		__syncthreads();
+		for (uint32_t i = t; i < bins; i += BB_THREADS) lh[i] = 0;
+		__syncthreads();
+		uint32_t where[BB_PER_THREAD];
+		uint64_t kept[KEEP ? BB_PER_THREAD : 1][W + 1];
+#pragma unroll
+		for (int i = 0; i < BB_PER_THREAD; i++) {
+			const uint64_t e = s0 + (uint64_t)i * BB_THREADS + t;
+			where[i] = 0xffffffffu;
+			if (e >= segEnd) continue;
+			uint64_t ew[W + 1];
+			bb_load_entry<W>(in.entries, e, ew);
+			if (in.holes && ew[W] == 0) continue;
+			Key<W> key;
+#pragma unroll
+			for (int q = 0; q < W; q++) key.w[q] = ew[q];
+			const uint32_t bin = (uint32_t)((key_hash<W>(key, kb) & (nb - 1)) >> shift) & mask;
+			where[i] = (bin << 16) | atomicAdd(&lh[bin], 1u);
+			if constexpr (KEEP) {
+#pragma unroll
+				for (int q = 0; q <= W; q++) kept[i][q] = ew[q];
+			}
+		}
+		__syncthreads();
+		for (uint32_t i = t; i < bins; i += BB_THREADS) {
+			const uint32_t c = lh[i];
+			if (!c) continue;
+			const uint64_t b = (seg << bits) + i;
+			const uint32_t r = atomicAdd(&fill[b], c);
+			if ((uint64_t)r + c > limit) { atomicOr(overflow, 1u); lbase[i] = ~0ull; }
+			else lbase[i] = b * stride + r;
+		}
+		__syncthreads();
+#pragma unroll
+		for (int i = 0; i < BB_PER_THREAD; i++) {
+			if (where[i] == 0xffffffffu) continue;
+			const unsigned long long base = lbase[where[i] >> 16];
+			if (base == ~0ull) continue;
+			if constexpr (KEEP) bb_store_entry<W>(out_entries, base + (where[i] & 0xffffu), kept[i]);
+			else {
+				uint64_t ew[W + 1];
+				bb_load_entry<W>(in.entries, s0 + (uint64_t)i * BB_THREADS + t, ew);
+				bb_store_entry<W>(out_entries, base + (where[i] & 0xffffu), ew);
+			}
+		}
+	}
+}
+
 static const int BB_GROUP_PER_THREAD = (BB_GROUP_CAP + BB_GROUP_THREADS - 1) / BB_GROUP_THREADS;
 template <int W> __host__ __device__ constexpr size_t bb_group_smem_bytes() { return (size_t)bb_group_cap<W>() * (8 * W + 8 + 2 + 2); }
 
 template <int W>
 __global__ __launch_bounds__(BB_GROUP_THREADS, W <= 2 ? 4 : 1)
 void bb_group_kernel(const uint64_t *entries, uint64_t *keys, uint32_t *vals, const uint64_t *gstart, const uint32_t *gcount, uint64_t n_groups, uint32_t gbits, uint32_t kb, uint64_t nb,
-                     uint64_t *start, uint64_t n_total, uint32_t *err) {
+                     uint64_t *start, uint64_t n_total, uint32_t *err, uint64_t in_stride, const uint32_t *overflow) {
+	if (overflow && *overflow) return;
 	extern __shared__ __attribute__((aligned(16))) uint8_t gsm[];
 	uint64_t *skeys = (uint64_t *)gsm;
 	constexpr uint32_t CAP = bb_group_cap<W>();
@@ -171,7 +235,7 @@
 	const int t = threadIdx.x;
 	const uint32_t nbk = 1u << gbits;
 	for (uint64_t G = blockIdx.x; G < n_groups; G += gridDim.x) {
-		const uint64_t base = gstart[G];
+		const uint64_t base = gstart[G], in_base = in_stride ? G * in_stride : base;
 		const uint32_t n = gcount[G];
 		__syncthreads();
 		if ((uint32_t)t < nbk) bcnt[t] = 0;
@@ -182,7 +246,7 @@
 		for (int u = 0; u < BB_GROUP_PER_THREAD; u++) {
 			const uint32_t i = (uint32_t)u * BB_GROUP_THREADS + t;
 			lb[u] = 0xffffffffu;
-			if (i < n) bb_load_entry<W>(entries, base + i, ew[u]);
+			if (i < n) bb_load_entry<W>(entries, in_base + i, ew[u]);
 		}
 #pragma unroll
 		for (int u = 0; u < BB_GROUP_PER_THREAD; u++) {
diff --git a/kmernator_amd/csrc/kmr_host.hpp b/kmernator_amd/csrc/kmr_host.hpp
--- a/kmernator_amd/csrc/kmr_host.hpp
+++ b/kmernator_amd/csrc/kmr_host.hpp
@@ -140,6 +140,9 @@
 	bool no_lut = false, no_narrow = false, no_l1_state = false, no_stream_lookups = false;
 	uint64_t long_list_chunks = 0;
 	uint64_t binned_min = 1ull << 18;
+	bool bb_fixed_bins = true;
+	double bb_slack_bins = 1.0, bb_slack_groups = 1.0;
+	bool bb_reload = false;
 	uint64_t twobit_piece_bases = 0;
 	uint64_t list_aim = 0;
 	bool pow2_lists = false;
@@ -197,6 +200,7 @@
 	uint32_t peer_uni_w = 0xffffffffu; bool peer_uni_mixed = false, peers_declare = false;
 	uint64_t xr_lo = 0, xr_hi = ~0ull;
 	uint64_t last_early_hi = 0, last_early_entries = 0;
+	int last_bb_path = 0; bool last_bb_fallback = false; uint32_t *bb_overflow = nullptr;
 	bool last_early_overflowed = false;
 	double last_score_ms = 0, last_select_ms = 0, last_write_ms = 0;
 	double last_dump_size_ms = 0, last_dump_write_ms = 0;
@@ -304,6 +308,7 @@
 uint64_t resize_buckets(uint64_t n);
 void quality_table(double P[256], unsigned minQ, unsigned startChar);
 int exclusive_scan(kmr_handle *h, const uint32_t *in, uint64_t n, uint64_t *out );
+int exclusive_scan_queue(kmr_handle *h, const uint32_t *in, uint64_t n, uint64_t *out );
 int num_cus(kmr_handle *h);
 struct ScoreDev { uint32_t *trim_offset, *trim_length; float *score; uint8_t *was_trimmed; };
 int score_reads_core(kmr_handle *h, const uint8_t *s_b, const uint64_t *s_o, uint64_t n_reads, double minimum_kmer_score, int scoring_type,
```
